# pouyaardehkhani/4DLangSplat

Measured on AMD Instinct MI355X. Metric: rasterizer fwd+bwd frames/sec @ 2M Gaussians, 1352x1014, 32-ch features, higher is better.
Workload: dtype f32; 1 GPU; S2M synthetic (BASELINE configs[2] per GPU; configs[3] batch split); gaussians=2000000, width=1352, height=1014, channels=32, global_batch=8, parallelism=dp1, pipeline=batched, binning=sort, early_views=2, order_on_side=True, num_rendered_mean=5615889

## Files before the change

4dlangsplat_amd/csrc/lsr_api.hip:

```cpp
#include <hip/hip_runtime.h>

#include <atomic>
#include <cstdio>
#include <cstring>
#include <mutex>
#include <string>
#include <vector>

#include "../../include/lsr.h"
#include "lsr_common.h"
#include "lsr_internal.h"

namespace {

thread_local std::string g_err;
std::atomic<int32_t> g_caller_api{0};

int fail(int code, const std::string& msg) {
    g_err = msg;
    return code;
}

#define LSR_HIP(expr)                                                                        \
    do {                                                                                     \
// ... 132 lines not shown
    BinningTb t;
    t.b = carve_binning(base, K, &head);
    Carver c(base);
    c.off = head;
    t.table = c.take<uint32_t>((size_t)lsr::tb_blocks((int)P) * ntiles);
    t.tmp = c.take<uint64_t>(K);
    if (bytes) *bytes = c.off;
    return t;
}

struct Img {
    uint2* ranges;
    uint32_t* tile_max;
    float* final_T;
    uint32_t* n_contrib;
    uint32_t* tile_order;
};
struct Grid { int x, y; size_t tiles() const { return (size_t)x * y; } };
Grid tile_grid(int W, int H) { return {(W + LSR_TILE_X - 1) / LSR_TILE_X, (H + LSR_TILE_Y - 1) / LSR_TILE_Y}; }
float focal(int extent, float tanfov) { return (float)extent / (2.0f * tanfov); }

Img carve_img(void* base, int W, int H, size_t* bytes) {
    const size_t ntiles = tile_grid(W, H).tiles();
    Carver c(base);
    Img m;
    m.ranges = c.take<uint2>(ntiles);
    m.tile_max = c.take<uint32_t>(ntiles);
    m.final_T = c.take<float>((size_t)W * H);
    m.n_contrib = c.take<uint32_t>((size_t)W * H);
    m.tile_order = c.take<uint32_t>(ntiles);
    if (bytes) *bytes = c.off;
    return m;
}

struct Scratch {
    float* acc_small;
    float* rec;
    uint8_t* flags;
};
Scratch carve_scratch(void* base, size_t P, size_t K, int recq, bool det, size_t* bytes) {
    Carver c(base);
    Scratch s{};
    if (det) {
        s.rec = c.take<float>(K * (size_t)recq);
        s.flags = c.take<uint8_t>(K);
    } else {
        s.acc_small = c.take<float>(P * lsr::ACC_PITCH);
    }
    if (bytes) *bytes = c.off;
    return s;
}

int tile_bits(int ntiles) {
    int b = 1;
    while ((1 << b) <= ntiles) ++b;
    return b;
}
bool tile_sort_in_b(int ntiles) { return ((tile_bits(ntiles) + 7) / 8) % 2 == 1; }
uint32_t* point_list(const Binning& b, Grid grid) { return tile_sort_in_b((int)grid.tiles()) ? b.val_b : b.val_a; }
int depth_sort_result_in_b() { return 0; }

int check_common(const lsr_settings* s, const lsr_fwd_in* in) {
    if (g_caller_api.load() != LSR_API_VERSION)
        return fail(LSR_EINVAL, "call lsr_require_api(LSR_API_VERSION) first: the caller must be built against lsr.h "
                                "version " + std::to_string(LSR_API_VERSION));
    if (!s || !in) return fail(LSR_EINVAL, "null settings or inputs");
    if (s->image_width <= 0 || s->image_height <= 0) return fail(LSR_EINVAL, "image size must be positive");
    if (s->image_width > 4095 * LSR_TILE_X || s->image_height > 4095 * LSR_TILE_Y)
        return fail(LSR_EINVAL, "image size exceeds 4095 tiles per axis");
    if (in->P < 0) return fail(LSR_EINVAL, "P must be >= 0");
    if (in->P >= (1 << 28)) return fail(LSR_EINVAL, "P must be < 2^28");
    if ((uint64_t)in->P * (uint64_t)(in->C > 16 ? in->C : 16) * 4u >= (1ull << 32))
        return fail(LSR_EINVAL, "P * max(C, 16) * 4 bytes must be < 2^32");
    if (!s->viewmatrix || !s->projmatrix || !s->bg || !s->campos)
        return fail(LSR_EINVAL, "viewmatrix, projmatrix, bg and campos are required");
    if (in->P > 0 && (!in->means3D || !in->opacities)) return fail(LSR_EINVAL, "means3D and opacities are required");
    if (in->P == 0) return LSR_OK;
    if ((in->shs == nullptr) == (in->colors_precomp == nullptr))
        return fail(LSR_EINVAL, "Please provide excatly one of either SHs or precomputed colors!");
    const bool sr = in->scales != nullptr || in->rotations != nullptr;
    if ((!(in->scales && in->rotations) && !in->cov3D_precomp) || (sr && in->cov3D_precomp))
        return fail(LSR_EINVAL, "Please provide exactly one of either scale/rotation pair or precomputed 3D covariance!");
    if (in->shs && (s->sh_degree < 0 || s->sh_degree > 3 || in->M < (s->sh_degree + 1) * (s->sh_degree + 1)))
        return fail(LSR_EINVAL, "sh_degree must be in [0, 3] and shs must hold (sh_degree + 1)^2 coefficients");
    if (in->C < 0 || in->C > 64) return fail(LSR_EINVAL, "language feature channels must be in [0, 64]");
    if (s->include_feature && in->C > 0 && in->P > 0 && !in->language_feature)
        return fail(LSR_EINVAL, "language_feature is required when C > 0");
    return LSR_OK;
}

enum : unsigned { SHARE_SIZE = 1, SHARE_SH_DEGREE = 2, SHARE_SCALE = 4, SHARE_FEATURE = 8 };
struct ViewRules { const char *no_views, *null_array; unsigned share; const char* share_msg; bool share_first; };
const char kArrays[] = "n_views >= 1 and the per-view arrays are required";
const ViewRules kPreprocessViews{kArrays, kArrays, SHARE_SIZE | SHARE_SH_DEGREE | SHARE_SCALE,
                                 "batched views must share the image size, sh_degree and scale_modifier", false};
const ViewRules kBinningViews{kArrays, kArrays, SHARE_SIZE, "batched views must share the image size", true};
const ViewRules kCompositeViews{kArrays, kArrays, SHARE_SIZE | SHARE_FEATURE,
                                "batched views must share the image size and include_feature", false};
const ViewRules kBackwardViews{"n_views must be >= 1", "null argument", SHARE_SCALE,
                               "all views must share scale_modifier", false};

bool shares(const lsr_settings* a, const lsr_settings* b, unsigned what) {
    return (!(what & SHARE_SIZE) || (a->image_width == b->image_width && a->image_height == b->image_height)) &&
           (!(what & SHARE_SH_DEGREE) || a->sh_degree == b->sh_degree) &&
           (!(what & SHARE_SCALE) || a->scale_modifier == b->scale_modifier) &&
           (!(what & SHARE_FEATURE) || (a->include_feature != 0) == (b->include_feature != 0));
}

template <typename Need>
int check_each_view(const ViewRules& rules, int32_t n_views, bool arrays, const lsr_settings* const* s,
                    const lsr_fwd_in* in, Need need) {
    if (n_views < 1) return fail(LSR_EINVAL, rules.no_views);
    if (!arrays) return fail(LSR_EINVAL, rules.null_array);
    for (int v = 0; v < n_views; ++v) {
        int rc = check_common(s[v], in);
        if (rc) return rc;
        if (rules.share_first && !shares(s[v], s[0], rules.share)) return fail(LSR_EINVAL, rules.share_msg);
        if ((rc = need(v))) return rc;
        if (!rules.share_first && !shares(s[v], s[0], rules.share)) return fail(LSR_EINVAL, rules.share_msg);
    }
    return LSR_OK;
}
int need_radii(int32_t n_views, lsr_fwd_out* const* out, int P) {
    for (int v = 0; v < n_views; ++v)
        if (!out[v] || (!out[v]->radii && P > 0)) return fail(LSR_EINVAL, "radii output is required");
    return LSR_OK;
}
int need_workspaces(const void* geom, const void* img, const void* binning, int64_t num_rendered) {
    if (!geom || !img || (num_rendered > 0 && !binning)) return fail(LSR_EINVAL, "workspaces are required");
    return LSR_OK;
}
int need_atomic_grads(const lsr_bwd_in* gin, const char* color_msg, const char* deterministic_msg) {
    if (!gin || !gin->dL_dout_color) return fail(LSR_EINVAL, color_msg);
    if (gin->deterministic) return fail(LSR_EINVAL, deterministic_msg);
    return LSR_OK;
}

void preprocess_shared(lsr::PreprocessArgs& a, const lsr_settings* s, const lsr_fwd_in* in) {
    const int W = s->image_width, H = s->image_height;
    const Grid grid = tile_grid(W, H);
    a.P = in->P; a.M = in->M; a.deg = s->sh_degree; a.W = W; a.H = H;
    a.grid_x = grid.x; a.grid_y = grid.y;
    a.scale_modifier = s->scale_modifier;
    a.means3D = in->means3D; a.scales = in->scales; a.rotations = in->rotations; a.opacities = in->opacities;
    a.shs = in->shs; a.colors_precomp = in->colors_precomp; a.cov3D_precomp = in->cov3D_precomp;
}
void preprocess_view(lsr::PreprocessView& v, const lsr_settings* s, const Geom& g, int* radii) {
    v.tanfovx = s->tanfovx; v.tanfovy = s->tanfovy;
    v.focal_x = focal(s->image_width, s->tanfovx);
    v.focal_y = focal(s->image_height, s->tanfovy);
    v.view = s->viewmatrix; v.proj = s->projmatrix; v.campos = s->campos;
    v.radii = radii; v.radius = g.radius; v.tiles = g.tiles; v.rect = g.rect; v.key = g.key_a; v.xy = g.xy;
    v.conic_o = g.conic_o; v.rgbd = g.rgbd; v.clamped = g.clamped;
    v.order = g.val_a;
    v.rank_counts = g.counts;
    v.acc = g.acc;
    v.clear.p[0] = g.total;
    v.clear.n[0] = 4;
}

uint32_t* mapped_counts(uint32_t* host_counts) {
    void* dptr = nullptr;
    if (hipHostGetDevicePointer(&dptr, host_counts, 0) == hipSuccess && dptr) return static_cast<uint32_t*>(dptr);
    (void)hipGetLastError();
    return nullptr;
}

int scan_counts(int nv, void* const* geom, int P, uint32_t* host_counts, uint32_t* mapped, hipStream_t st, bool debug) {
    lsr::ScanSeg sc[lsr::LSR_MAX_VIEWS] = {};
    const uint32_t* total[lsr::LSR_MAX_VIEWS];
    for (int k = 0; k < nv; ++k) {
        Geom g = carve_geom(geom[k], (size_t)P, nullptr);
        sc[k] = lsr::ScanSeg{g.counts, g.offsets, g.total, reinterpret_cast<uint32_t*>(g.scan_tmp), (size_t)P};
        total[k] = g.total;
        if (mapped) {
            sc[k].host_total = mapped + 2 * k;
            host_counts[2 * k + 1] = 0;
        }
    }
    uint32_t wrote;
    {
        PhaseTimer t(LSR_PHASE_INSTANCE_SCAN, st);
        wrote = lsr::exclusive_scan_batch(sc, nv, st);
    }
    LSR_LAUNCHED("instance scan", st, debug);
    for (int k = 0; k < nv; ++k)
        if (!((wrote >> k) & 1u))
            LSR_HIP(hipMemcpyAsync(host_counts + 2 * k, total[k], 2 * sizeof(uint32_t), hipMemcpyDeviceToHost, st));
    return LSR_OK;
}

struct BinBatch { int P, W, H; Grid grid; size_t ntiles; hipStream_t st; bool debug; };
struct BinView { Geom g; Img m; size_t K; void* binning; };
template <typename Launch>
int bin_views(int32_t n_views, const lsr_settings* const* s, const lsr_fwd_in* in, void* const* geom,
              void* const* binning, void* const* img, const int64_t* num_rendered, lsr_stream_t stream,
              size_t max_tiles, const char* too_many_tiles, Launch launch) {
    int rc = check_each_view(kBinningViews, n_views, s && geom && binning && img && num_rendered, s, in, [&](int v) {
        return need_workspaces(geom[v], img[v], binning[v], num_rendered[v]);
    });
    if (rc) return rc;
    const Grid grid = tile_grid(s[0]->image_width, s[0]->image_height);
    const BinBatch c{in->P, s[0]->image_width, s[0]->image_height, grid, grid.tiles(),
                     reinterpret_cast<hipStream_t>(stream), s[0]->debug != 0};
    if (c.ntiles > max_tiles) return fail(LSR_EINVAL, too_many_tiles);
    for (int v0 = 0; v0 < n_views; v0 += lsr::LSR_MAX_VIEWS) {
        const int nv = std::min(n_views - v0, lsr::LSR_MAX_VIEWS);
        BinView bv[lsr::LSR_MAX_VIEWS];
        int ne = 0;
        for (int v = v0; v < v0 + nv; ++v) {
            const size_t K = (size_t)num_rendered[v];
            Geom g = carve_geom(geom[v], (size_t)(c.P > 0 ? c.P : 1), nullptr);
            Img m = carve_img(img[v], c.W, c.H, nullptr);
            if (K == 0) {
                LSR_HIP(hipMemsetAsync(m.ranges, 0, sizeof(uint2) * c.ntiles, c.st));
                LSR_HIP(hipMemsetAsync(m.tile_max, 0, sizeof(uint32_t) * c.ntiles, c.st));
                continue;
            }
            bv[ne++] = BinView{g, m, K, binning[v]};
        }
        if (ne == 0) continue;
        if ((rc = launch(c, bv, ne))) return rc;
    }
    return LSR_OK;
}

void render_bwd_view(lsr::RenderBwdArgs& r, const lsr_settings* s, const lsr_fwd_in* in, const lsr_bwd_in* gin,
                     const Geom& g, const Binning& b, const Img& m) {
    const int W = s->image_width, H = s->image_height;
    const Grid grid = tile_grid(W, H);
    r.W = W; r.H = H; r.grid_x = grid.x; r.grid_y = grid.y; r.C = in->C; r.include_feature = s->include_feature;
    r.ranges = m.ranges; r.point_list = point_list(b, grid);
    r.xy = g.xy; r.conic_o = g.conic_o; r.rgbd = g.rgbd;
    r.rect = g.rect; r.inst_off = g.inst_off;
    r.lang = in->language_feature;
    r.lang_split = in->C == 32 ? in->language_feature_split : nullptr;
    r.bg = s->bg; r.final_T = m.final_T; r.n_contrib = m.n_contrib;
    r.tile_max_contrib = m.tile_max; r.tile_order = m.tile_order;
    r.dL_dcolor = gin->dL_dout_color; r.dL_dlang = gin->dL_dout_language_feature; r.dL_ddepth = gin->dL_dout_depth;
}

}

extern "C" {
namespace {
int check_views(int32_t n_views, const lsr_settings* const* s, const lsr_fwd_in* in, void* const* geom) {
    return check_each_view(kPreprocessViews, n_views, s && geom, s, in,
                           [&](int v) { return geom[v] ? LSR_OK : fail(LSR_EINVAL, "geom workspaces are required"); });
}

int preprocess_rows(int32_t n_views, int32_t row0, int32_t row1, int counts_tiles, const lsr_settings* const* s,
                    const lsr_fwd_in* in, lsr_fwd_out* const* out, void* const* geom, hipStream_t st) {
    const int P = in->P;
    if (row1 == row0) return LSR_OK;
    for (int v0 = 0; v0 < n_views; v0 += lsr::LSR_MAX_VIEWS) {
        const int nv = std::min(n_views - v0, lsr::LSR_MAX_VIEWS);
        lsr::PreprocessArgs a{};
        preprocess_shared(a, s[v0], in);
        a.nv = nv;
        a.row0 = row0;
        a.P = row1;
        a.counts_tiles = counts_tiles;
        for (int k = 0; k < nv; ++k) {
            Geom g = carve_geom(geom[v0 + k], (size_t)P, nullptr);
            preprocess_view(a.v[k], s[v0 + k], g, out[v0 + k]->radii);
        }
        {
            PhaseTimer t(LSR_PHASE_PREPROCESS, st);
            lsr::launch_preprocess(a, st);
        }
        LSR_LAUNCHED("preprocess", st, s[v0]->debug);
    }
    return LSR_OK;
}

int depth_order_views(int32_t n_views, const lsr_settings* const* s, const lsr_fwd_in* in, void* const* geom,
                      uint32_t* host_counts, uint32_t* mapped, hipStream_t st) {
    const int P = in->P;
    for (int v0 = 0; v0 < n_views; v0 += lsr::LSR_MAX_VIEWS) {
        const int nv = std::min(n_views - v0, lsr::LSR_MAX_VIEWS);
        lsr::SortSeg ss[lsr::LSR_MAX_VIEWS] = {};
        for (int k = 0; k < nv; ++k) {
            Geom g = carve_geom(geom[v0 + k], (size_t)P, nullptr);
            ss[k] = lsr::SortSeg{g.key_a, g.val_a, g.key_b, g.val_b, g.sort_tmp, g.total + 3,
                                 lsr::SortGather{g.rect, g.counts, g.rect_sorted}, (size_t)P};
            ss[k].vals_c = g.offsets;
        }
        {
            PhaseTimer t(LSR_PHASE_DEPTH_SORT, st);
            if (lsr::radix_sort_batch(ss, nv, 0, 32, st) != depth_sort_result_in_b())
                return fail(LSR_EHIP, "internal: depth sort batch or parity");
        }
        LSR_LAUNCHED("depth sort", st, s[v0]->debug);
        int rc = scan_counts(nv, geom + v0, P, host_counts + 2 * v0, mapped ? mapped + 2 * v0 : nullptr, st,
                             s[v0]->debug);
        if (rc) return rc;
    }
    return LSR_OK;
}

int instance_scan_views(int32_t n_views, const lsr_fwd_in* in, void* const* geom, uint32_t* host_counts,
                        uint32_t* mapped, hipStream_t st, bool debug) {
    for (int v0 = 0; v0 < n_views; v0 += lsr::LSR_MAX_VIEWS) {
        int rc = scan_counts(std::min(n_views - v0, lsr::LSR_MAX_VIEWS), geom + v0, in->P, host_counts + 2 * v0,
                             mapped ? mapped + 2 * v0 : nullptr, st, debug);
        if (rc) return rc;
    }
    return LSR_OK;
}
}
}

namespace {
int preprocess_and_order(int32_t n_views, int32_t n_ordered, const lsr_settings* const* s, const lsr_fwd_in* in,
                         lsr_fwd_out* const* out, void* const* geom, uint32_t* host_counts, bool map_counts,
                         hipStream_t st) {
    if (in->P == 0) {
        for (int v = 0; v < 2 * n_ordered; ++v) host_counts[v] = 0;
        return LSR_OK;
    }
    int rc = preprocess_rows(n_views, 0, in->P, 0, s, in, out, geom, st);
    if (rc || n_ordered == 0) return rc;
    return depth_order_views(n_ordered, s, in, geom, host_counts, map_counts ? mapped_counts(host_counts) : nullptr, st);
}

int preprocess_rows_checked(int32_t n_views, int32_t row0, int32_t row1, int counts_tiles, const lsr_settings* const* s,
                            const lsr_fwd_in* in, lsr_fwd_out* const* out, void* const* geom, lsr_stream_t stream) {
    int rc = check_views(n_views, s, in, geom);
    if (rc) return rc;
    if (!out || row0 < 0 || row1 < row0 || row1 > in->P || row0 % 256 != 0)
        return fail(LSR_EINVAL, "0 <= row0 <= row1 <= P with row0 a multiple of 256, and the outputs are required");
    if ((rc = need_radii(n_views, out, in->P))) return rc;
    return preprocess_rows(n_views, row0, row1, counts_tiles, s, in, out, geom, reinterpret_cast<hipStream_t>(stream));
}

int count_views(int32_t n_views, const lsr_settings* const* s, const lsr_fwd_in* in, void* const* geom,
                uint32_t* host_counts, lsr_stream_t stream, bool depth_sort) {
    int rc = check_views(n_views, s, in, geom);
    if (rc) return rc;
    if (!host_counts) return fail(LSR_EINVAL, "host_counts is required");
    if (in->P == 0) {
        for (int v = 0; v < 2 * n_views; ++v) host_counts[v] = 0;
        return LSR_OK;
    }
    hipStream_t st = reinterpret_cast<hipStream_t>(stream);
    uint32_t* mapped = mapped_counts(host_counts);
    return depth_sort ? depth_order_views(n_views, s, in, geom, host_counts, mapped, st)
                      : instance_scan_views(n_views, in, geom, host_counts, mapped, st, s[0]->debug);
}

lsr::PreprocessBwdViewsArgs preprocess_bwd_args(const lsr_settings* s, const lsr_fwd_in* in, const lsr_bwd_out* gout,
                                                size_t r0, int n, int nv) {
    lsr::PreprocessBwdViewsArgs a{};
    a.P = n; a.M = in->M; a.nv = nv; a.scale_modifier = s->scale_modifier;
    a.means3D = in->means3D + 3 * r0;
    a.scales = in->scales ? in->scales + 3 * r0 : nullptr;
    a.rotations = in->rotations ? in->rotations + 4 * r0 : nullptr;
    a.shs = in->shs ? in->shs + (size_t)in->M * 3 * r0 : nullptr;
    a.cov3D_precomp = in->cov3D_precomp ? in->cov3D_precomp + 6 * r0 : nullptr;
    a.dopacity = gout->dL_dopacity;
    a.dmeans3D = gout->dL_dmeans3D; a.dmeans2D = gout->dL_dmeans2D; a.dcolors = gout->dL_dcolors;
    a.dcov3D = gout->dL_dcov3D; a.dsh = in->shs ? gout->dL_dsh : nullptr; a.dscales = gout->dL_dscales;
    a.drots = gout->dL_drotations;
    return a;
}
void view_cam(lsr::ViewCam& c, const lsr_settings* s, const Geom& g, const float* acc_small, size_t r0) {
    c.view = s->viewmatrix; c.proj = s->projmatrix; c.campos = s->campos;
    c.tanfovx = s->tanfovx; c.tanfovy = s->tanfovy;
    c.focal_x = focal(s->image_width, s->tanfovx);
    c.focal_y = focal(s->image_height, s->tanfovy);
    c.deg = s->sh_degree;
    c.tiles = g.tiles + r0; c.clamped = g.clamped + r0;
    c.acc_small = acc_small + lsr::ACC_PITCH * r0;
}

}

extern "C" {

int lsr_version(void) { return LSR_API_VERSION; }
int lsr_require_api(int32_t caller_version) {
    if (caller_version != LSR_API_VERSION)
        return fail(LSR_EINVAL, "lsr.h version mismatch: caller " + std::to_string(caller_version) + ", library " +
                                    std::to_string(LSR_API_VERSION));
    g_caller_api.store(caller_version);
    return LSR_OK;
}
const char* lsr_last_error(void) { return g_err.c_str(); }

int64_t lsr_geom_bytes(int32_t P) {
    size_t b;
    carve_geom(nullptr, (size_t)(P > 0 ? P : 1), &b);
    return (int64_t)b;
}
int64_t lsr_binning_bytes(int64_t K) {
    size_t b;
    carve_binning(nullptr, (size_t)(K > 0 ? K : 1), &b);
    return (int64_t)b;
}
int64_t lsr_binning_bytes_tb(int64_t K, int32_t P, int32_t W, int32_t H) {
    if (W <= 0 || H <= 0 || P < 0) return -1;
    size_t b;
    carve_binning_tb(nullptr, (size_t)(K > 0 ? K : 1), (size_t)(P > 0 ? P : 1), tile_grid(W, H).tiles(), &b);
    return (int64_t)b;
}
int64_t lsr_img_bytes(int32_t W, int32_t H) {
    size_t b;
    carve_img(nullptr, W, H, &b);
    return (int64_t)b;
}
int64_t lsr_backward_bytes(int32_t P, int64_t K, int32_t C, int32_t deterministic) {
    size_t b;
    carve_scratch(nullptr, (size_t)(P > 0 ? P : 1), (size_t)(K > 0 ? K : 1), lsr::record_floats(C > 0 ? C : 0),
                  deterministic != 0, &b);
    return (int64_t)b;
}

int lsr_forward_preprocess_async(const lsr_settings* s, const lsr_fwd_in* in, lsr_fwd_out* out, void* geom,
                                 uint32_t* host_count, lsr_stream_t stream) {
    int rc = check_common(s, in);
    if (rc) return rc;
    if ((rc = need_radii(1, &out, in->P))) return rc;
    if (!geom || !host_count) return fail(LSR_EINVAL, "geom workspace and host_count are required");
    return preprocess_and_order(1, 1, &s, in, &out, &geom, host_count, false, reinterpret_cast<hipStream_t>(stream));
}

int lsr_forward_preprocess_views_split_async(int32_t n_views, int32_t n_ordered, const lsr_settings* const* s,
                                             const lsr_fwd_in* in, lsr_fwd_out* const* out, void* const* geom,
                                             uint32_t* host_counts, lsr_stream_t stream) {
    int rc = check_views(n_views, s, in, geom);
    if (rc) return rc;
    if (!out || (n_ordered > 0 && !host_counts) || n_ordered < 0 || n_ordered > n_views)
        return fail(LSR_EINVAL, "0 <= n_ordered <= n_views, the outputs and host_counts are required");
    if ((rc = need_radii(n_views, out, in->P))) return rc;
    return preprocess_and_order(n_views, n_ordered, s, in, out, geom, host_counts, true,
                                reinterpret_cast<hipStream_t>(stream));
}

int lsr_forward_preprocess_views_rows_async(int32_t n_views, int32_t row0, int32_t row1, const lsr_settings* const* s,
                                            const lsr_fwd_in* in, lsr_fwd_out* const* out, void* const* geom,
                                            lsr_stream_t stream) {
    return preprocess_rows_checked(n_views, row0, row1, 0, s, in, out, geom, stream);
}

int lsr_forward_preprocess_views_tb_async(int32_t n_views, int32_t row0, int32_t row1, const lsr_settings* const* s,
                                          const lsr_fwd_in* in, lsr_fwd_out* const* out, void* const* geom,
                                          lsr_stream_t stream) {
    return preprocess_rows_checked(n_views, row0, row1, 1, s, in, out, geom, stream);
}

int lsr_forward_instance_scan_views_async(int32_t n_views, const lsr_settings* const* s, const lsr_fwd_in* in,
                                          void* const* geom, uint32_t* host_counts, lsr_stream_t stream) {
    return count_views(n_views, s, in, geom, host_counts, stream, false);
}

int lsr_forward_depth_order_views_async(int32_t n_views, const lsr_settings* const* s, const lsr_fwd_in* in,
                                        void* const* geom, uint32_t* host_counts, lsr_stream_t stream) {
    return count_views(n_views, s, in, geom, host_counts, stream, true);
}

int lsr_forward_preprocess_views_async(int32_t n_views, const lsr_settings* const* s, const lsr_fwd_in* in,
                                       lsr_fwd_out* const* out, void* const* geom, uint32_t* host_counts,
                                       lsr_stream_t stream) {
    if (!host_counts) return fail(LSR_EINVAL, "host_counts is required");
    return lsr_forward_preprocess_views_split_async(n_views, n_views, s, in, out, geom, host_counts, stream);
}

int lsr_forward_preprocess(const lsr_settings* s, const lsr_fwd_in* in, lsr_fwd_out* out, void* geom,
                           int64_t* num_rendered, lsr_stream_t stream) {
    if (!num_rendered) return fail(LSR_EINVAL, "geom workspace and num_rendered are required");
    uint32_t tot[2] = {0, 0};
    int rc = lsr_forward_preprocess_async(s, in, out, geom, tot, stream);
    if (rc) return rc;
    LSR_HIP(hipStreamSynchronize(reinterpret_cast<hipStream_t>(stream)));
    *num_rendered = (int64_t)tot[0];
    return LSR_OK;
}

int lsr_forward_binning(const lsr_settings* s, const lsr_fwd_in* in, void* geom, void* binning, void* img,
                        int64_t num_rendered, lsr_stream_t stream) {
    return lsr_forward_binning_views(1, &s, in, &geom, &binning, &img, &num_rendered, stream);
}

int lsr_forward_binning_views(int32_t n_views, const lsr_settings* const* s, const lsr_fwd_in* in, void* const* geom,
                              void* const* binning, void* const* img, const int64_t* num_rendered,
                              lsr_stream_t stream) {
    const auto emit_and_sort = [](const BinBatch& c, const BinView* bv, int ne) {
        const size_t ntiles = c.ntiles;
        hipStream_t st = c.st;
        lsr::EmitBatch eb{};
        eb.P = c.P; eb.grid_x = c.grid.x; eb.grid_y = c.grid.y; eb.W = c.W; eb.H = c.H;
        lsr::SortSeg ss[lsr::LSR_MAX_VIEWS] = {};
        for (int k = 0; k < ne; ++k) {
            const Geom& g = bv[k].g;
            const Img& m = bv[k].m;
            Binning b = carve_binning(bv[k].binning, bv[k].K, nullptr);
            lsr::EmitView& e = eb.v[k];
            e.order = g.val_a; e.offsets = g.offsets; e.counts = g.counts; e.rect_sorted = g.rect_sorted;
            e.xy = g.xy; e.conic_o = g.conic_o; e.keys = b.key_a; e.vals = b.val_a;
            e.clear.p[0] = reinterpret_cast<uint32_t*>(m.ranges);
            e.clear.n[0] = (uint32_t)(2 * ntiles);
            e.clear.even[0] = 0xFFFFFFFFu;
            e.clear.p[1] = m.tile_max;
            e.clear.n[1] = (uint32_t)ntiles;
            ss[k] = lsr::SortSeg{b.key_a, b.val_a, b.key_b, b.val_b, b.sort_tmp, b.kept,
                                 lsr::SortGather{nullptr, nullptr, nullptr}, bv[k].K, m.ranges, (uint32_t)ntiles};
        }
        {
            PhaseTimer t(LSR_PHASE_EMIT, st);
            lsr::launch_emit_instances(eb, ne, st);
        }
        LSR_LAUNCHED("emit", st, c.debug);
        {
            PhaseTimer t(LSR_PHASE_TILE_SORT, st);
            const int in_b = lsr::radix_sort_batch(ss, ne, 0, tile_bits((int)ntiles), st);
            if (in_b < 0 || (in_b == 1) != tile_sort_in_b((int)ntiles))
                return fail(LSR_EHIP, "internal: tile sort batch or parity");
        }
        LSR_LAUNCHED("tile sort", st, c.debug);
        return LSR_OK;
    };
    return bin_views(n_views, s, in, geom, binning, img, num_rendered, stream, SIZE_MAX, nullptr, emit_and_sort);
}

int lsr_forward_binning_views_tb(int32_t n_views, const lsr_settings* const* s, const lsr_fwd_in* in, void* const* geom,
                                 void* const* binning, void* const* img, const int64_t* num_rendered,
                                 lsr_stream_t stream) {
    const auto bucket = [](const BinBatch& c, const BinView* bv, int ne) {
        lsr::TbBatch tb{};
        tb.P = c.P; tb.grid_x = c.grid.x; tb.grid_y = c.grid.y; tb.W = c.W; tb.H = c.H; tb.ntiles = (int)c.ntiles;
        for (int k = 0; k < ne; ++k) {
            const Geom& g = bv[k].g;
            const Img& m = bv[k].m;
            BinningTb b = carve_binning_tb(bv[k].binning, bv[k].K, (size_t)c.P, c.ntiles, nullptr);
            lsr::TbView& t = tb.v[k];
            t.counts = g.counts; t.offsets = g.offsets; t.rect = g.rect; t.xy = g.xy; t.conic_o = g.conic_o;
            t.depth = g.key_a;
            t.table = b.table;
            t.tile_total = m.tile_order;
            t.tile_start = m.tile_max;
            t.ranges = m.ranges;
            t.keys = reinterpret_cast<uint64_t*>(b.b.key_a);
            t.tmp = b.tmp;
            t.words = point_list(b.b, c.grid);
            t.tile_max = m.tile_max;
        }
        {
            PhaseTimer t(LSR_PHASE_TILE_SORT, c.st);
            const hipError_t e = lsr::launch_tile_bucket_binning(tb, ne, c.st);
            if (e != hipSuccess)
                return fail(LSR_EHIP, std::string("tile-bucket binning: dynamic LDS attribute: ") + hipGetErrorString(e));
        }
        LSR_LAUNCHED("tile-bucket binning", c.st, c.debug);
        return LSR_OK;
    };
    return bin_views(n_views, s, in, geom, binning, img, num_rendered, stream, 12288,
                     "tile-bucket binning: more than 12288 tiles (use lsr_forward_binning_views)", bucket);
}

int lsr_forward_composite(const lsr_settings* s, const lsr_fwd_in* in, lsr_fwd_out* out, const void* geom,
                          const void* binning, void* img, int64_t num_rendered, lsr_stream_t stream) {
    lsr_fwd_out* o[1] = {out};
    return lsr_forward_composite_views(1, &s, in, o, &geom, &binning, &img, &num_rendered, stream);
}

int lsr_forward_composite_views(int32_t n_views, const lsr_settings* const* s, const lsr_fwd_in* in,
                                lsr_fwd_out* const* out, const void* const* geom, const void* const* binning,
                                void* const* img, const int64_t* num_rendered, lsr_stream_t stream) {
    int rc = check_each_view(kCompositeViews, n_views, s && out && geom && binning && img && num_rendered, s, in, [&](int v) {
        if (!out[v] || !out[v]->out_color || !out[v]->out_depth) return fail(LSR_EINVAL, "color and depth outputs are required");
        if (in->C > 0 && !out[v]->out_language_feature)
            return fail(LSR_EINVAL, "language feature output is required when C > 0");
        return need_workspaces(geom[v], img[v], binning[v], num_rendered[v]);
    });
    if (rc) return rc;
    hipStream_t st = reinterpret_cast<hipStream_t>(stream);
    const int P = in->P, W = s[0]->image_width, H = s[0]->image_height, C = in->C;
    const Grid grid = tile_grid(W, H);
    for (int v0 = 0; v0 < n_views; v0 += lsr::LSR_MAX_VIEWS) {
        const int nv = std::min(n_views - v0, lsr::LSR_MAX_VIEWS);
        lsr::RenderFwdArgs r[lsr::LSR_MAX_VIEWS] = {};
        for (int k = 0; k < nv; ++k) {
            const int v = v0 + k;
            const size_t K = (size_t)num_rendered[v];
            Geom g = carve_geom(const_cast<void*>(geom[v]), (size_t)(P > 0 ? P : 1), nullptr);
            Binning b = carve_binning(const_cast<void*>(binning[v]), K > 0 ? K : 1, nullptr);
            Img m = carve_img(img[v], W, H, nullptr);
            lsr::RenderFwdArgs& a = r[k];
            a.W = W; a.H = H; a.grid_x = grid.x; a.grid_y = grid.y; a.C = C; a.include_feature = s[v]->include_feature;
            a.ranges = m.ranges; a.point_list = K > 0 ? point_list(b, grid) : nullptr;
            a.xy = g.xy; a.conic_o = g.conic_o; a.rgbd = g.rgbd;
            a.lang = in->language_feature;
            a.lang_split = in->C == 32 ? in->language_feature_split : nullptr;
            a.bg = s[v]->bg; a.final_T = m.final_T; a.n_contrib = m.n_contrib;
            a.tile_max_contrib = m.tile_max; a.tile_order = m.tile_order;
            a.out_color = out[v]->out_color; a.out_lang = out[v]->out_language_feature;
            a.out_depth = out[v]->out_depth;
            if (C > 0 && !s[v]->include_feature)
                LSR_HIP(hipMemsetAsync(out[v]->out_language_feature, 0, sizeof(float) * (size_t)C * W * H, st));
        }
        {
// ... 256 lines not shown
```

4dlangsplat_amd/csrc/lsr_internal.h:

```cpp
#pragma once
#include <hip/hip_runtime.h>
#include <stdint.h>

namespace lsr {

constexpr int ACC_PITCH = 16;

struct ClearList {
    uint32_t* p[4];
    uint32_t n[4];
    uint32_t even[4];
};

constexpr int LSR_MAX_VIEWS = 8;
__device__ __forceinline__ void clear_words(const ClearList& c) {
    const uint32_t t = blockIdx.x * blockDim.x + threadIdx.x, stride = gridDim.x * blockDim.x;
#pragma unroll
    for (int k = 0; k < 4; ++k)
        for (uint32_t i = t; i < c.n[k]; i += stride) c.p[k][i] = (i & 1u) ? 0u : c.even[k];
}

__host__ __device__ __forceinline__ uint2 rect_pack(uint32_t x0, uint32_t y0, uint32_t x1, uint32_t y1, uint32_t map) {
    return make_uint2(x0 | y0 << 12 | (map & 0xFFu) << 24, x1 | y1 << 12 | (map >> 8) << 24);
}
__host__ __device__ __forceinline__ void rect_unpack(uint2 r, uint32_t& x0, uint32_t& y0, uint32_t& x1, uint32_t& y1) {
    x0 = r.x & 0xFFFu; y0 = (r.x >> 12) & 0xFFFu; x1 = r.y & 0xFFFu; y1 = (r.y >> 12) & 0xFFFu;
}
__host__ __device__ __forceinline__ uint32_t rect_quad_map(uint2 r) { return (r.x >> 24) | (r.y >> 24) << 8; }
__host__ __device__ __forceinline__ bool rect_small(uint32_t x0, uint32_t y0, uint32_t x1, uint32_t y1) {
    return x1 - x0 <= 2 && y1 - y0 <= 2;
}
__host__ __device__ __forceinline__ uint32_t rect_tile_mask(uint32_t map) {
    return ((map & 0x33u) ? 1u : 0u) | ((map & 0xCCu) ? 2u : 0u) | ((map & 0x3300u) ? 4u : 0u) |
           ((map & 0xCC00u) ? 8u : 0u);
}
__host__ __device__ __forceinline__ uint32_t rect_count(uint2 r) {
    uint32_t x0, y0, x1, y1;
    rect_unpack(r, x0, y0, x1, y1);
    if ((x1 - x0) * (y1 - y0) > 0 && rect_small(x0, y0, x1, y1)) return __builtin_popcount(rect_tile_mask(rect_quad_map(r)));
    return (x1 - x0) * (y1 - y0);
}
__host__ __device__ __forceinline__ uint32_t rect_local_index(uint2 r, uint32_t tx, uint32_t ty) {
    uint32_t x0, y0, x1, y1;
    rect_unpack(r, x0, y0, x1, y1);
    if (rect_small(x0, y0, x1, y1))
        return __builtin_popcount(rect_tile_mask(rect_quad_map(r)) & ((1u << (2 * (ty - y0) + (tx - x0))) - 1u));
    return (ty - y0) * (x1 - x0) + (tx - x0);
}

struct PreprocessView {
    float tanfovx, tanfovy, focal_x, focal_y;
    const float* view;
    const float* proj;
    const float* campos;
    int* radii;
    int* radius;
    uint32_t* tiles;
    uint2* rect;
    uint32_t* key;
    float2* xy;
    float4* conic_o;
    float4* rgbd;
    uint8_t* clamped;
    uint32_t* order;
    uint32_t* rank_counts;
    float4* acc;
    ClearList clear;
};
struct PreprocessArgs {
    int P, M, deg, W, H, grid_x, grid_y, nv;
    int row0;
    int counts_tiles;
    float scale_modifier;
    const float* means3D;
    const float* scales;
    const float* rotations;
    const float* opacities;
    const float* shs;
    const float* colors_precomp;
    const float* cov3D_precomp;
    PreprocessView v[LSR_MAX_VIEWS];
};

struct ViewCam {
    const float* view;
    const float* proj;
    const float* campos;
    float tanfovx, tanfovy, focal_x, focal_y;
    int deg;
    const uint32_t* tiles;
    const uint8_t* clamped;
    const float* acc_small;
};
struct PreprocessBwdViewsArgs {
    int P, M, nv;
    float scale_modifier;
    const float* means3D;
    const float* scales;
    const float* rotations;
    const float* shs;
    const float* cov3D_precomp;
    ViewCam cam[LSR_MAX_VIEWS];
    float* dopacity;
    float* dmeans3D;
    float* dmeans2D;
    float* dcolors;
    float* dcov3D;
    float* dsh;
    float* dscales;
    float* drots;
    const float* rec;
    const uint8_t* flags;
    const uint32_t* inst_off;
    int recq;
    int deterministic;
};
void launch_preprocess_bwd_views(const PreprocessBwdViewsArgs& a, bool accumulate, bool one_view, hipStream_t st);

void launch_language_split(int P, const float* lang, uint16_t* out, hipStream_t st);
void launch_radii_max(int P, int n, const int* const* radii, int* out, bool accumulate, hipStream_t st);

struct RenderFwdArgs {
    int W, H, grid_x, grid_y, C, include_feature;
    uint2* ranges;
    const uint32_t* point_list;
    const float2* xy;
    const float4* conic_o;
    const float4* rgbd;
    const float* lang;
    const uint16_t* lang_split;
    const float* bg;
    float* final_T;
    uint32_t* n_contrib;
    uint32_t* tile_max_contrib;
    uint32_t* tile_order;
    float* out_color;
    float* out_lang;
    float* out_depth;
};

struct RenderBwdArgs {
    int W, H, grid_x, grid_y, C, include_feature;
    const uint2* ranges;
    const uint32_t* point_list;
    const float2* xy;
    const float4* conic_o;
    const float4* rgbd;
    const uint2* rect;
    const uint32_t* inst_off;
    const float* lang;
    const uint16_t* lang_split;
    const float* bg;
    const float* final_T;
    const uint32_t* n_contrib;
    const uint32_t* tile_max_contrib;
    uint32_t* tile_order;
    const float* dL_dcolor;
    const float* dL_dlang;
    const float* dL_ddepth;
    float* rec;
    uint8_t* flags;
    int recq;
    int deterministic;
    float* acc_small;
    float* acc_lang;
};

struct RenderFwdBatch { RenderFwdArgs v[LSR_MAX_VIEWS]; };
struct RenderBwdBatch { RenderBwdArgs v[LSR_MAX_VIEWS]; };
void launch_render_fwd_views(const RenderFwdArgs* a, int n, hipStream_t st);
void launch_render_bwd_wave_views(const RenderBwdArgs* a, int n, hipStream_t st);

inline int lang_pad(int C) { return C == 0 ? 0 : C <= 4 ? 4 : C <= 8 ? 8 : C <= 16 ? 16 : C <= 32 ? 32 : 64; }
inline int record_floats(int C) { return 12 + lang_pad(C); }

constexpr int DEF_MAX_LAYERS = 4;
constexpr int DEF_HEADS = 6;
constexpr int DEF_W2ROWS = 64;
constexpr int DEF_LANG_MODE_PASS = 0, DEF_LANG_MODE_RESIDUAL = 1, DEF_LANG_MODE_NORESNET = 2,
              DEF_LANG_MODE_DISCRETE = 3;
struct DeformArgs {
    int P;
    int n_scales, nlayers;
    uint32_t heads;
    int apply_rotation, lang_mode, lang_dim, centers, lang_in;
    const float* means3D;
    const float* time;
    const float* aabb;
    const float* planes;
    int64_t poff[24];
    int pw[24], ph[24];
    const __bf16 *wf_h[DEF_MAX_LAYERS], *wf_l[DEF_MAX_LAYERS];
    const __bf16 *w1_h[DEF_HEADS], *w1_l[DEF_HEADS];
    const __bf16 *w2_h[DEF_HEADS], *w2_l[DEF_HEADS];
    const float* b_feat[DEF_MAX_LAYERS];
    const float* b1[DEF_HEADS];
    const float* b2[DEF_HEADS];
    const float* in[5];
    const float* lang;
    float* out[5];
    float* out_lang;
    float* out_coff;
};
void launch_deform_fwd(const DeformArgs& a, hipStream_t st);
enum PackKind { PACK_PLANE = 0, PACK_WEIGHT = 1, PACK_WEIGHT_T = 2 };
struct PackJob {
    int kind, a, b, c, d;
    uint32_t first_block;
    const float* src;
    void* hi;
    __bf16* lo;
};
constexpr int PACK_MAX_JOBS = 64;
struct PackBatch { PackJob j[PACK_MAX_JOBS]; int n; };
void launch_pack_batch(PackJob* jobs, int n, hipStream_t st);

struct DeformBwdArgs {
    DeformArgs f;
    const __bf16 *wft_h[DEF_MAX_LAYERS], *wft_l[DEF_MAX_LAYERS];
    const __bf16 *w1t_h[DEF_HEADS], *w1t_l[DEF_HEADS];
    const __bf16 *w2t_h[DEF_HEADS], *w2t_l[DEF_HEADS];
    const float* up[5];
    const float* up_lang;
    const float* up_coff;
    float* d_means3D;
    float* d_rotations;
    float* d_lang;
    float* dplanes;
    int64_t plane_stride;
    int replicas;
    float* trow;
    int64_t toff[24];
    int64_t trow_stride;
    int trow_reps;
    float* sX;
    float* sA[DEF_MAX_LAYERS];
    float* sdH[DEF_MAX_LAYERS];
    float* sG_rot;
    float* sG_coff;
    float* daabb;
    float* daabb_part;
};
constexpr int DEF_AABB_SLOTS = 64;
void launch_deform_bwd_a(const DeformBwdArgs& a, hipStream_t st);
struct HeadWgradJob {
    const float* G;
    const __bf16 *w1_h, *w1_l;
    const float* b1;
    const __bf16 *w2t_h, *w2t_l;
    const __bf16 *w2_h, *w2_l;
    float *dW1, *db1, *dW2, *db2;
    int nout;
};
constexpr int DEF_WGRAD_MAX_JOBS = DEF_HEADS;
struct HeadWgradArgs {
    HeadWgradJob job[DEF_WGRAD_MAX_JOBS];
    const float* A;
    int P, rows_per_block;
};
void launch_head_wgrad(const HeadWgradArgs& a, int njobs, hipStream_t st);
struct AtbJob {
    const float* L;
    const float* R;
    float* C;
    float* bias;
    int M, N;
};
constexpr int LSR_ATB_MAX_JOBS = 20;
struct AtbArgs {
    AtbJob job[LSR_ATB_MAX_JOBS];
    int P;
    int rows_per_block;
};
void launch_atb(const AtbArgs& a, int njobs, hipStream_t st);
constexpr int DEF_UNPACK_MAX = 24;
struct UnpackBatch {
    const float* src;
    int64_t off[DEF_UNPACK_MAX];
    float* dst[DEF_UNPACK_MAX];
    int H[DEF_UNPACK_MAX], W[DEF_UNPACK_MAX];
    int block0[DEF_UNPACK_MAX + 1];
    int n, replicas;
    int64_t stride;
    const float* daabb_part;
    float* daabb;
    const float* trow;
    int64_t toff[DEF_UNPACK_MAX];
    int64_t trow_stride;
    int trow_reps;
    const float* time0;
};
void launch_unpack_planes(const UnpackBatch& u, hipStream_t st);

struct LangDeformArgs {
    int P, lang_dim, time_pe, kin, residual;
    const float* lang;
    const float* time;
    const __bf16 *w_h[3], *w_l[3];
    const float* b[3];
    float* out_lang;
    const __bf16 *wt_h[3], *wt_l[3];
    const float* up_lang;
    float* d_lang;
    float *sU0, *sU1, *sU2;
    float *sdv, *sdZ2, *sdZ1;
};
void launch_lang_deform_fwd(const LangDeformArgs& a, hipStream_t st);
void launch_lang_deform_bwd(const LangDeformArgs& a, hipStream_t st);

void launch_preprocess(const PreprocessArgs& a, hipStream_t st);
void launch_reduce_lang(int P, int C, int cpad, int recq, const float* rec, const uint8_t* flags,
                        const uint32_t* inst_off, const uint32_t* tiles, float* dlang, bool accumulate, hipStream_t st);
void launch_mark_visible(int P, const float* means3D, const float* view, uint8_t* present, hipStream_t st);

size_t scan_temp_bytes(size_t n);
void exclusive_scan_u32(const uint32_t* in, uint32_t* out, size_t n, uint32_t* total, void* temp, hipStream_t st);
constexpr int SCAN_SEG_TILES = 4096;
struct ScanSeg {
    const uint32_t* in;
    uint32_t* out;
    uint32_t* total;
    uint32_t* partials;
    size_t n;
    uint32_t* host_total = nullptr;
};
struct ScanBatch { ScanSeg s[LSR_MAX_VIEWS]; };
uint32_t exclusive_scan_batch(const ScanSeg* segs, int nseg, hipStream_t st);
size_t radix_temp_bytes(size_t n);
struct SortGather {
    const uint2* rect;
    uint32_t* counts;
    uint2* rect_sorted;
};
struct SortSeg {
    uint32_t *keys_a, *vals_a, *keys_b, *vals_b;
    void* temp;
    uint32_t* kept;
    SortGather gather;
    size_t n;
    uint2* ranges;
    uint32_t nranges;
    uint32_t* vals_c;
};
struct SortBatch { SortSeg s[LSR_MAX_VIEWS]; };
int radix_sort_batch(const SortSeg* segs, int nseg, int begin_bit, int end_bit, hipStream_t st);
bool radix_sort_pairs(uint32_t* keys_a, uint32_t* vals_a, uint32_t* keys_b, uint32_t* vals_b, size_t n,
                      int begin_bit, int end_bit, void* temp, hipStream_t st, uint32_t* kept = nullptr,
                      const SortGather* gather = nullptr, uint32_t* vals_c = nullptr);

constexpr uint32_t PL_ID_MASK = 0x0FFFFFFFu;
constexpr int PL_QUAD_SHIFT = 28;
struct EmitView {
    const uint32_t* order;
    const uint32_t* offsets;
    const uint32_t* counts;
    const uint2* rect_sorted;
    const float2* xy;
    const float4* conic_o;
    uint32_t* keys;
    uint32_t* vals;
    ClearList clear;
};
struct EmitBatch {
    int P, grid_x, grid_y, W, H;
    EmitView v[LSR_MAX_VIEWS];
};
void launch_emit_instances(const EmitBatch& eb, int nv, hipStream_t st);
void launch_scatter_inst_off(int P, const uint32_t* order, const uint32_t* offsets, const uint32_t* counts,
                             uint32_t* inst_off, hipStream_t st);
struct TbView {
    const uint32_t* counts;
    const uint32_t* offsets;
    const uint2* rect;
    const float2* xy;
    const float4* conic_o;
    const uint32_t* depth;
    uint32_t* table;
    uint32_t* tile_total;
    uint32_t* tile_start;
    uint2* ranges;
    uint64_t* keys;
    uint64_t* tmp;
    uint32_t* words;
    uint32_t* tile_max;
};
struct TbBatch {
    int P, grid_x, grid_y, W, H, ntiles;
    TbView v[LSR_MAX_VIEWS];
};
int tb_blocks(int P);
hipError_t launch_tile_bucket_binning(const TbBatch& tb, int nv, hipStream_t st);

void launch_render_bwd(const RenderBwdArgs& a, hipStream_t st);
void launch_render_fwd_wave_views(const RenderFwdArgs* a, int n, hipStream_t st);
void launch_render_fwd_wave_mfma_views(const RenderFwdArgs* a, int n, hipStream_t st);

}
```

4dlangsplat_amd/csrc/preprocess.hip:

```cpp
#include "lsr_common.h"
#include "lsr_internal.h"

namespace lsr {

struct m3 { float m[3][3]; };

__device__ __forceinline__ m3 mul(const m3& a, const m3& b) {
    m3 o;
#pragma unroll
    for (int c = 0; c < 3; ++c)
#pragma unroll
        for (int r = 0; r < 3; ++r)
            o.m[c][r] = a.m[0][r] * b.m[c][0] + a.m[1][r] * b.m[c][1] + a.m[2][r] * b.m[c][2];
    return o;
}
__device__ __forceinline__ m3 tr(const m3& a) {
    m3 o;
#pragma unroll
    for (int c = 0; c < 3; ++c)
#pragma unroll
        for (int r = 0; r < 3; ++r) o.m[c][r] = a.m[r][c];
    return o;
}
__device__ __forceinline__ m3 quat_R(float4 q) {
    const float r = q.x, x = q.y, y = q.z, z = q.w;
    m3 R;
    R.m[0][0] = 1.0f - 2.0f * (y * y + z * z); R.m[0][1] = 2.0f * (x * y - r * z); R.m[0][2] = 2.0f * (x * z + r * y);
    R.m[1][0] = 2.0f * (x * y + r * z); R.m[1][1] = 1.0f - 2.0f * (x * x + z * z); R.m[1][2] = 2.0f * (y * z - r * x);
    R.m[2][0] = 2.0f * (x * z - r * y); R.m[2][1] = 2.0f * (y * z + r * x); R.m[2][2] = 1.0f - 2.0f * (x * x + y * y);
    return R;
}
__device__ __forceinline__ m3 zero3() {
    m3 o;
#pragma unroll
    for (int c = 0; c < 3; ++c)
#pragma unroll
        for (int r = 0; r < 3; ++r) o.m[c][r] = 0.0f;
    return o;
}

__device__ __forceinline__ void cov3d(float3 s, float mod, float4 q, float* cov) {
    m3 S = zero3();
    S.m[0][0] = mod * s.x; S.m[1][1] = mod * s.y; S.m[2][2] = mod * s.z;
    const m3 Rm = quat_R(q);
    const m3 M = mul(S, Rm);
    const m3 Sig = mul(tr(M), M);
    cov[0] = Sig.m[0][0]; cov[1] = Sig.m[0][1]; cov[2] = Sig.m[0][2];
    cov[3] = Sig.m[1][1]; cov[4] = Sig.m[1][2]; cov[5] = Sig.m[2][2];
}

__device__ __forceinline__ m3 view_W(const float* __restrict__ v) {
    m3 W;
    W.m[0][0] = v[0]; W.m[0][1] = v[4]; W.m[0][2] = v[8];
    W.m[1][0] = v[1]; W.m[1][1] = v[5]; W.m[1][2] = v[9];
    W.m[2][0] = v[2]; W.m[2][1] = v[6]; W.m[2][2] = v[10];
    return W;
}
__device__ __forceinline__ m3 sym3(const float* c) {
    m3 V;
    V.m[0][0] = c[0]; V.m[0][1] = c[1]; V.m[0][2] = c[2];
    V.m[1][0] = c[1]; V.m[1][1] = c[3]; V.m[1][2] = c[4];
    V.m[2][0] = c[2]; V.m[2][1] = c[4]; V.m[2][2] = c[5];
    return V;
}

__constant__ float SH_C0 = 0.28209479177387814f;
__constant__ float SH_C1 = 0.4886025119029199f;
__constant__ float SH_C2[5] = {1.0925484305920792f, -1.0925484305920792f, 0.31539156525252005f,
                               -1.0925484305920792f, 0.5462742152960396f};
__constant__ float SH_C3[7] = {-0.5900435899266435f, 2.890611442640554f, -0.4570457994644658f,
                               0.3731763325901154f, -0.4570457994644658f, 1.445305721320277f,
                               -0.5900435899266435f};

template <int M3>
__device__ __forceinline__ void stage_rows(float* __restrict__ lds, const float* __restrict__ src, int rows) {
    if constexpr (M3 > 0) {
        constexpr int SP = M3 + 1;
        const int n = rows * M3;
        for (int e = threadIdx.x; e < n; e += blockDim.x) {
            const int r = e / M3, c = e - r * M3;
            lds[r * SP + c] = src[e];
        }
    }
}

template <int MS>
struct GaussIn {
    float3 p;
    float op;
    float c3[6];
    float sh[MS > 0 ? 3 * MS : 1];
};
__device__ __forceinline__ float3 load_mean(const PreprocessArgs& a, int i) {
    return make_float3(a.means3D[3 * i], a.means3D[3 * i + 1], a.means3D[3 * i + 2]);
}
__device__ __forceinline__ void load_cov3d(const PreprocessArgs& a, int i, float (&c3)[6]) {
    if (a.cov3D_precomp) {
#pragma unroll
        for (int k = 0; k < 6; ++k) c3[k] = a.cov3D_precomp[6 * (size_t)i + k];
    } else {
        const float3 s = make_float3(a.scales[3 * i], a.scales[3 * i + 1], a.scales[3 * i + 2]);
        const float4 q = reinterpret_cast<const float4*>(a.rotations)[i];
        cov3d(s, a.scale_modifier, q, c3);
    }
}
template <int MS, int N>
__device__ __forceinline__ void load_sh(const PreprocessArgs& a, int i, float (&shr)[N]) {
    constexpr int M3 = MS * 3;
    const float* src = a.shs + (size_t)i * M3;
    if (M3 % 4 == 0 && (reinterpret_cast<uintptr_t>(src) & 15) == 0) {
#pragma unroll
        for (int q = 0; q < M3 / 4; ++q) {
            const float4 t = reinterpret_cast<const float4*>(src)[q];
            shr[4 * q] = t.x; shr[4 * q + 1] = t.y; shr[4 * q + 2] = t.z; shr[4 * q + 3] = t.w;
        }
    } else {
#pragma unroll
        for (int q = 0; q < M3; ++q) shr[q] = src[q];
    }
}
template <int MS>
__device__ __forceinline__ void load_gauss(const PreprocessArgs& a, int i, GaussIn<MS>& g) {
    g.p = load_mean(a, i);
    g.op = a.opacities[i];
    load_cov3d(a, i, g.c3);
    if constexpr (MS > 0) {
        if (a.shs && !a.colors_precomp) load_sh<MS>(a, i, g.sh);
    }
}

template <int MS, bool PRE>
__device__ __forceinline__ bool preprocess_one(const PreprocessArgs& a, const PreprocessView& v, const GaussIn<MS>& g,
                                               int i) {
    v.radii[i] = 0;
    v.radius[i] = 0;
    v.tiles[i] = 0;
    v.rect[i] = make_uint2(0u, 0u);
    v.clamped[i] = 0;
    if (v.order) v.order[i] = (uint32_t)i;
    if (v.rank_counts) v.rank_counts[i] = 0u;
    if (v.key) v.key[i] = 0xFFFFFFFFu;
    const float3 p = PRE ? g.p : load_mean(a, i);
    const float4 ph = xform4x4(v.proj, p);
    const float3 pv = xform4x3(v.view, p);
    if (pv.z <= 0.2f) return false;
    const float pw = 1.0f / (ph.w + 0.0000001f);
    const float3 pp = make_float3(ph.x * pw, ph.y * pw, ph.z * pw);

    float c3[6];
    if constexpr (PRE) {
#pragma unroll
        for (int k = 0; k < 6; ++k) c3[k] = g.c3[k];
    } else {
        load_cov3d(a, i, c3);
    }
    float3 t = pv;
    const float limx = 1.3f * v.tanfovx, limy = 1.3f * v.tanfovy;
    const float txtz = t.x / t.z, tytz = t.y / t.z;
    t.x = fminf(limx, fmaxf(-limx, txtz)) * t.z;
    t.y = fminf(limy, fmaxf(-limy, tytz)) * t.z;
    m3 J = zero3();
    J.m[0][0] = v.focal_x / t.z; J.m[0][2] = -(v.focal_x * t.x) / (t.z * t.z);
    J.m[1][1] = v.focal_y / t.z; J.m[1][2] = -(v.focal_y * t.y) / (t.z * t.z);
    const m3 T = mul(view_W(v.view), J);
    const m3 V = sym3(c3);
    const m3 A = mul(tr(T), tr(V));
    const m3 cv = mul(A, T);
    const float ca = cv.m[0][0] + 0.3f, cb = cv.m[0][1], cc = cv.m[1][1] + 0.3f;
    const float det = ca * cc - cb * cb;
    if (det == 0.0f) return false;
    const float det_inv = 1.0f / det;
    const float4 conic = make_float4(cc * det_inv, -cb * det_inv, ca * det_inv, PRE ? g.op : a.opacities[i]);
    const float mid = 0.5f * (ca + cc);
    const float l1 = mid + sqrtf(fmaxf(0.1f, mid * mid - det));
    const float l2 = mid - sqrtf(fmaxf(0.1f, mid * mid - det));
    const int radius = (int)ceilf(3.0f * sqrtf(fmaxf(l1, l2)));
    const float2 pix = make_float2(ndc2pix(pp.x, a.W), ndc2pix(pp.y, a.H));
    int2 rmin, rmax;
    tile_rect(pix, radius, a.grid_x, a.grid_y, rmin, rmax);
    if ((rmax.y - rmin.y) * (rmax.x - rmin.x) == 0) return false;
    const float thr = skip_power(conic.w);
    int ntiles = 0;
    int2 cmin = make_int2(0, 0), cmax = make_int2(0, 0);
    if (thr <= 0.0f) {
        const float rr = (float)radius + 16.0f;
        const float mt = (fabsf(conic.x) + fabsf(conic.z) + 2.0f * fabsf(conic.y)) * rr * rr;
        const float qm = -2.0f * thr + 1e-6f * mt + 1e-4f;
        const float hx = sqrtf(qm * ca) + 0.01f, hy = sqrtf(qm * cc) + 0.01f;
        cmin.x = max(rmin.x, (int)floorf((pix.x - hx) / (float)LSR_TILE_X));
        cmin.y = max(rmin.y, (int)floorf((pix.y - hy) / (float)LSR_TILE_Y));
        cmax.x = min(rmax.x, (int)floorf((pix.x + hx) / (float)LSR_TILE_X) + 1);
        cmax.y = min(rmax.y, (int)floorf((pix.y + hy) / (float)LSR_TILE_Y) + 1);
        if (cmax.x > cmin.x && cmax.y > cmin.y) ntiles = (cmax.x - cmin.x) * (cmax.y - cmin.y);
        else cmin = cmax = make_int2(0, 0);
    }

    float rgb[3];
    if (a.colors_precomp) {
        rgb[0] = a.colors_precomp[3 * i]; rgb[1] = a.colors_precomp[3 * i + 1]; rgb[2] = a.colors_precomp[3 * i + 2];
    } else {
        float3 dir = make_float3(p.x - v.campos[0], p.y - v.campos[1], p.z - v.campos[2]);
        const float len = sqrtf(dir.x * dir.x + dir.y * dir.y + dir.z * dir.z);
        dir.x = dir.x / len; dir.y = dir.y / len; dir.z = dir.z / len;
        float shr[48];
        if constexpr (MS > 0) {
            if constexpr (PRE) {
#pragma unroll
                for (int q = 0; q < 3 * MS; ++q) shr[q] = g.sh[q];
            } else {
                load_sh<MS>(a, i, shr);
            }
        }
        const float* sh = MS > 0 ? shr : a.shs + (size_t)i * a.M * 3;
        uint8_t cl = 0;
        const int deg = a.deg;
#pragma unroll
        for (int ch = 0; ch < 3; ++ch) {
#define SHc(k) sh[(k) * 3 + ch]
            float res = SH_C0 * SHc(0);
            if (deg > 0) {
                const float x = dir.x, y = dir.y, z = dir.z;
                res = res - SH_C1 * y * SHc(1) + SH_C1 * z * SHc(2) - SH_C1 * x * SHc(3);
                if (deg > 1) {
                    const float xx = x * x, yy = y * y, zz = z * z, xy = x * y, yz = y * z, xz = x * z;
                    res = res + SH_C2[0] * xy * SHc(4) + SH_C2[1] * yz * SHc(5) +
                          SH_C2[2] * (2.0f * zz - xx - yy) * SHc(6) + SH_C2[3] * xz * SHc(7) +
                          SH_C2[4] * (xx - yy) * SHc(8);
                    if (deg > 2) {
                        res = res + SH_C3[0] * y * (3.0f * xx - yy) * SHc(9) + SH_C3[1] * xy * z * SHc(10) +
                              SH_C3[2] * y * (4.0f * zz - xx - yy) * SHc(11) +
                              SH_C3[3] * z * (2.0f * zz - 3.0f * xx - 3.0f * yy) * SHc(12) +
                              SH_C3[4] * x * (4.0f * zz - xx - yy) * SHc(13) + SH_C3[5] * z * (xx - yy) * SHc(14) +
                              SH_C3[6] * x * (xx - 3.0f * yy) * SHc(15);
                    }
                }
            }
#undef SHc
            res = res + 0.5f;
            cl |= (res < 0.0f ? 1 : 0) << ch;
            rgb[ch] = res < 0.0f ? 0.0f : res;
        }
        v.clamped[i] = cl;
    }
    v.radii[i] = radius;
    v.radius[i] = radius;
    uint32_t qmap = 0;
    if (ntiles > 0 && cmax.x - cmin.x <= 2 && cmax.y - cmin.y <= 2) {
        const EmitSplat es = emit_splat(pix, conic);
        const float ex = emit_margin(es);
        for (int ty = cmin.y; ty < cmax.y; ++ty)
#pragma unroll
            for (int band = 0; band < 2; ++band) {
                bool ok;
                float xmin, xmax;
                emit_band(es, ty * LSR_TILE_Y + 8 * band, a.H, ex, ok, xmin, xmax);
                for (int tx = cmin.x; tx < cmax.x; ++tx)
#pragma unroll
                    for (int col = 0; col < 2; ++col)
                        qmap |= emit_col_hit(es, ok, xmin, xmax, tx * LSR_TILE_X + 8 * col, a.W)
                                    ? 1u << (8 * (ty - cmin.y) + 4 * band + 2 * (tx - cmin.x) + col) : 0u;
            }
    }
    const uint2 rc = rect_pack((uint32_t)cmin.x, (uint32_t)cmin.y, (uint32_t)cmax.x, (uint32_t)cmax.y, qmap);
    v.rect[i] = rc;
    v.tiles[i] = rect_count(rc);
    if (v.rank_counts && a.counts_tiles) v.rank_counts[i] = rect_count(rc);
    if (v.key) v.key[i] = __float_as_uint(pv.z);
    v.xy[i] = pix;
    v.conic_o[i] = conic;
    v.rgbd[i] = make_float4(rgb[0], rgb[1], rgb[2], pv.z);
    return ntiles > 0;
}

__device__ __forceinline__ void zero_acc_rows(float4* acc, bool rect, int i) {
    if (!acc) return;
    const uint64_t m = __ballot(rect);
    if (m == 0) return;
    const int ln = threadIdx.x & 63;
    float4* w = acc + (size_t)(i - ln) * (ACC_PITCH / 4);
#pragma unroll
    for (int q = 0; q < ACC_PITCH / 4; ++q) {
        const int e = q * 64 + ln;
        if ((m >> (e / (ACC_PITCH / 4))) & 1) w[e] = make_float4(0.0f, 0.0f, 0.0f, 0.0f);
    }
}

template <int MS, bool MULTI>
__global__ void __launch_bounds__(256) k_preprocess(PreprocessArgs a) {
    const int i = a.row0 + blockIdx.x * blockDim.x + threadIdx.x;
    GaussIn<MS> g;
    if constexpr (!MULTI) {
        clear_words(a.v[0].clear);
        const bool rect = i < a.P && preprocess_one<MS, false>(a, a.v[0], g, i);
        zero_acc_rows(a.v[0].acc, rect, i);
    } else {
        const bool ok = i < a.P;
        if (ok) load_gauss<MS>(a, i, g);
        for (int k = 0; k < a.nv; ++k) {
            const PreprocessView& v = a.v[k];
            clear_words(v.clear);
            const bool rect = ok && preprocess_one<MS, true>(a, v, g, i);
            zero_acc_rows(v.acc, rect, i);
        }
    }
}

void launch_preprocess(const PreprocessArgs& a, hipStream_t st) {
    if (a.P <= a.row0 || a.nv <= 0) return;
    const dim3 grid((a.P - a.row0 + 255) / 256), block(256);
#define LSR_PP(MS)                                                                   \
    do {                                                                             \
        if (a.nv > 1) hipLaunchKernelGGL((k_preprocess<MS, true>), grid, block, 0, st, a);  \
        else hipLaunchKernelGGL((k_preprocess<MS, false>), grid, block, 0, st, a);          \
    } while (0)
    switch ((a.shs && !a.colors_precomp) ? a.M : 0) {
        case 1: LSR_PP(1); break;
        case 4: LSR_PP(4); break;
        case 9: LSR_PP(9); break;
        case 16: LSR_PP(16); break;
        default: LSR_PP(0); break;
    }
#undef LSR_PP
}

__global__ void k_mark_visible(int P, const float* __restrict__ means3D, const float* __restrict__ view,
                               uint8_t* __restrict__ present) {
    const int i = blockIdx.x * blockDim.x + threadIdx.x;
    if (i >= P) return;
    const float3 p = make_float3(means3D[3 * i], means3D[3 * i + 1], means3D[3 * i + 2]);
    present[i] = xform4x3(view, p).z > 0.2f;
}
struct RadiiMaxArgs { const int* r[LSR_MAX_VIEWS]; };
__global__ void __launch_bounds__(256) k_radii_max(int P, int n, RadiiMaxArgs ra, int* __restrict__ out, int accumulate) {
    const int i4 = blockIdx.x * 256 + threadIdx.x, i = 4 * i4;
    if (i >= P) return;
    if (i + 4 <= P) {
        int4 m = accumulate ? reinterpret_cast<const int4*>(out)[i4] : make_int4(0, 0, 0, 0);
        for (int v = 0; v < n; ++v) {
            const int4 x = reinterpret_cast<const int4*>(ra.r[v])[i4];
            m = make_int4(max(m.x, x.x), max(m.y, x.y), max(m.z, x.z), max(m.w, x.w));
        }
        reinterpret_cast<int4*>(out)[i4] = m;
    } else {
        for (int k = i; k < P; ++k) {
            int m = accumulate ? out[k] : 0;
            for (int v = 0; v < n; ++v) m = max(m, ra.r[v][k]);
            out[k] = m;
        }
    }
}
void launch_radii_max(int P, int n, const int* const* radii, int* out, bool accumulate, hipStream_t st) {
    for (int v0 = 0; v0 < n; v0 += LSR_MAX_VIEWS) {
        RadiiMaxArgs ra{};
        const int nv = n - v0 < LSR_MAX_VIEWS ? n - v0 : LSR_MAX_VIEWS;
        for (int k = 0; k < nv; ++k) ra.r[k] = radii[v0 + k];
        hipLaunchKernelGGL(k_radii_max, dim3((unsigned)((P + 1023) / 1024)), dim3(256), 0, st, P, nv, ra, out,
                           (accumulate || v0 > 0) ? 1 : 0);
    }
}

void launch_mark_visible(int P, const float* means3D, const float* view, uint8_t* present, hipStream_t st) {
    if (P == 0) return;
    hipLaunchKernelGGL(k_mark_visible, dim3((P + 255) / 256), dim3(256), 0, st, P, means3D, view, present);
}

__device__ void cov2d_bwd(float3 mean, const float* c3, float fx, float fy, float tanfovx, float tanfovy,
                          const float* __restrict__ view, float3 dconic, float3& dmean, float* dcov) {
#pragma clang fp contract(fast)
    float3 t = xform4x3(view, mean);
    const float limx = 1.3f * tanfovx, limy = 1.3f * tanfovy;
    const float txtz = t.x / t.z, tytz = t.y / t.z;
    t.x = fminf(limx, fmaxf(-limx, txtz)) * t.z;
    t.y = fminf(limy, fmaxf(-limy, tytz)) * t.z;
    const float x_grad_mul = (txtz < -limx || txtz > limx) ? 0.0f : 1.0f;
    const float y_grad_mul = (tytz < -limy || tytz > limy) ? 0.0f : 1.0f;
    const float tz = __builtin_amdgcn_rcpf(t.z), tz2 = tz * tz, tz3 = tz2 * tz;
    const float J00 = fx * tz, J11 = fy * tz, J02 = -(fx * t.x) * tz2, J12 = -(fy * t.y) * tz2;
    float u0[3], u1[3], Vu0[3], Vu1[3];
#pragma unroll
    for (int r = 0; r < 3; ++r) {
        u0[r] = view[4 * r] * J00 + view[4 * r + 2] * J02;
        u1[r] = view[4 * r + 1] * J11 + view[4 * r + 2] * J12;
    }
    const float V[3][3] = {{c3[0], c3[1], c3[2]}, {c3[1], c3[3], c3[4]}, {c3[2], c3[4], c3[5]}};
#pragma unroll
    for (int r = 0; r < 3; ++r) {
        Vu0[r] = V[r][0] * u0[0] + V[r][1] * u0[1] + V[r][2] * u0[2];
        Vu1[r] = V[r][0] * u1[0] + V[r][1] * u1[1] + V[r][2] * u1[2];
    }
    const float a = u0[0] * Vu0[0] + u0[1] * Vu0[1] + u0[2] * Vu0[2] + 0.3f;
    const float b = u0[0] * Vu1[0] + u0[1] * Vu1[1] + u0[2] * Vu1[2];
    const float c = u1[0] * Vu1[0] + u1[1] * Vu1[1] + u1[2] * Vu1[2] + 0.3f;
    const float denom = a * c - b * b;
    float dL_da = 0.0f, dL_db = 0.0f, dL_dc = 0.0f;
    const float denom2inv = __builtin_amdgcn_rcpf((denom * denom) + 0.0000001f);
    if (denom2inv != 0.0f) {
        dL_da = denom2inv * (-c * c * dconic.x + 2.0f * b * c * dconic.y + (denom - a * c) * dconic.z);
        dL_dc = denom2inv * (-a * a * dconic.z + 2.0f * a * b * dconic.y + (denom - a * c) * dconic.x);
        dL_db = denom2inv * 2.0f * (b * c * dconic.x - (denom + 2.0f * b * b) * dconic.y + a * b * dconic.z);
    }
    dcov[0] = u0[0] * u0[0] * dL_da + u0[0] * u1[0] * dL_db + u1[0] * u1[0] * dL_dc;
    dcov[3] = u0[1] * u0[1] * dL_da + u0[1] * u1[1] * dL_db + u1[1] * u1[1] * dL_dc;
    dcov[5] = u0[2] * u0[2] * dL_da + u0[2] * u1[2] * dL_db + u1[2] * u1[2] * dL_dc;
    dcov[1] = 2.0f * u0[0] * u0[1] * dL_da + (u0[0] * u1[1] + u0[1] * u1[0]) * dL_db + 2.0f * u1[0] * u1[1] * dL_dc;
    dcov[2] = 2.0f * u0[0] * u0[2] * dL_da + (u0[0] * u1[2] + u0[2] * u1[0]) * dL_db + 2.0f * u1[0] * u1[2] * dL_dc;
    dcov[4] = 2.0f * u0[2] * u0[1] * dL_da + (u0[1] * u1[2] + u0[2] * u1[1]) * dL_db + 2.0f * u1[1] * u1[2] * dL_dc;
    float dT0[3], dT1[3];
#pragma unroll
    for (int k = 0; k < 3; ++k) {
        dT0[k] = 2.0f * Vu0[k] * dL_da + Vu1[k] * dL_db;
        dT1[k] = 2.0f * Vu1[k] * dL_dc + Vu0[k] * dL_db;
    }
    const float dJ00 = view[0] * dT0[0] + view[4] * dT0[1] + view[8] * dT0[2];
    const float dJ02 = view[2] * dT0[0] + view[6] * dT0[1] + view[10] * dT0[2];
    const float dJ11 = view[1] * dT1[0] + view[5] * dT1[1] + view[9] * dT1[2];
    const float dJ12 = view[2] * dT1[0] + view[6] * dT1[1] + view[10] * dT1[2];
    const float dtx = x_grad_mul * -fx * tz2 * dJ02;
    const float dty = y_grad_mul * -fy * tz2 * dJ12;
    const float dtz = -fx * tz2 * dJ00 - fy * tz2 * dJ11 + (2.0f * fx * t.x) * tz3 * dJ02 + (2.0f * fy * t.y) * tz3 * dJ12;
    dmean.x = view[0] * dtx + view[1] * dty + view[2] * dtz;
    dmean.y = view[4] * dtx + view[5] * dty + view[6] * dtz;
    dmean.z = view[8] * dtx + view[9] * dty + view[10] * dtz;
}

__device__ void cov3d_bwd(float3 sc, float mod, float4 q, const float* dcov, float3& dscale, float4& drot) {
#pragma clang fp contract(fast)
    const float r = q.x, x = q.y, y = q.z, z = q.w;
    const m3 Rm = quat_R(q);
    const float s[3] = {mod * sc.x, mod * sc.y, mod * sc.z};
    m3 S = zero3();
    S.m[0][0] = s[0]; S.m[1][1] = s[1]; S.m[2][2] = s[2];
    const m3 M = mul(S, Rm);
    m3 dS;
    dS.m[0][0] = dcov[0]; dS.m[0][1] = 0.5f * dcov[1]; dS.m[0][2] = 0.5f * dcov[2];
    dS.m[1][0] = 0.5f * dcov[1]; dS.m[1][1] = dcov[3]; dS.m[1][2] = 0.5f * dcov[4];
    dS.m[2][0] = 0.5f * dcov[2]; dS.m[2][1] = 0.5f * dcov[4]; dS.m[2][2] = dcov[5];
    m3 M2;
#pragma unroll
    for (int c = 0; c < 3; ++c)
#pragma unroll
        for (int k = 0; k < 3; ++k) M2.m[c][k] = 2.0f * M.m[c][k];
    const m3 dM = mul(M2, dS);
    const m3 Rt = tr(Rm);
    m3 d = tr(dM);
    float ds[3];
#pragma unroll
    for (int k = 0; k < 3; ++k) ds[k] = (Rt.m[k][0] * d.m[k][0] + Rt.m[k][1] * d.m[k][1] + Rt.m[k][2] * d.m[k][2]) * mod;
    dscale = make_float3(ds[0], ds[1], ds[2]);
#pragma unroll
    for (int k = 0; k < 3; ++k) { d.m[0][k] *= s[0]; d.m[1][k] *= s[1]; d.m[2][k] *= s[2]; }
    drot.x = 2.0f * z * (d.m[0][1] - d.m[1][0]) + 2.0f * y * (d.m[2][0] - d.m[0][2]) + 2.0f * x * (d.m[1][2] - d.m[2][1]);
    drot.y = 2.0f * y * (d.m[1][0] + d.m[0][1]) + 2.0f * z * (d.m[2][0] + d.m[0][2]) + 2.0f * r * (d.m[1][2] - d.m[2][1]) -
             4.0f * x * (d.m[2][2] + d.m[1][1]);
    drot.z = 2.0f * x * (d.m[1][0] + d.m[0][1]) + 2.0f * r * (d.m[2][0] - d.m[0][2]) + 2.0f * z * (d.m[1][2] + d.m[2][1]) -
             4.0f * y * (d.m[2][2] + d.m[0][0]);
// ... 354 lines not shown
```

4dlangsplat_amd/csrc/sort.hip:

```cpp
#include "lsr_common.h"
#include "lsr_internal.h"

namespace lsr {

constexpr int SCAN_ITEMS = 8;
constexpr int SCAN_TILE = 256 * SCAN_ITEMS;

static inline size_t align_up(size_t x, size_t a) { return (x + a - 1) / a * a; }

__device__ __forceinline__ void block_exclusive_scan8(uint32_t (&v)[SCAN_ITEMS], uint32_t* s_wave,
                                                      uint32_t& block_total) {
    const int lane = threadIdx.x & 63, wave = threadIdx.x >> 6;
    uint32_t local = 0;
#pragma unroll
    for (int i = 0; i < SCAN_ITEMS; ++i) { const uint32_t x = v[i]; v[i] = local; local += x; }
    uint32_t inc = local;
#pragma unroll
    for (int o = 1; o < 64; o <<= 1) {
        const uint32_t t = __shfl_up(inc, o);
        if (lane >= o) inc += t;
    }
    if (lane == 63) s_wave[wave] = inc;
    __syncthreads();
    uint32_t wave_off = 0, total = 0;
// ... 271 lines not shown
    const uint64_t lt = lanemask_lt();
    const size_t base = (size_t)blockIdx.x * (256 * IT) + (size_t)wave * (64 * IT);
    uint32_t key[IT];
#pragma unroll
    for (int r = 0; r < IT; ++r) {
        const size_t idx = base + (size_t)r * 64 + lane;
        key[r] = idx < n ? keys[idx] : 0u;
    }
    uint32_t kmin = 0xFFFFFFFFu, kmax = 0u;
#pragma unroll
    for (int r = 0; r < IT; ++r) {
        const bool valid = base + (size_t)r * 64 + lane < n && !(drop && key[r] == 0xFFFFFFFFu);
        if (valid) {
            kmin = min(kmin, key[r]);
            kmax = max(kmax, key[r]);
        }
        const uint32_t d = ((key[r] - pd.kbase) >> pd.shift) & mask;
        const uint64_t peers = match_digit(d, valid, pd.nbits);
        if (valid && (peers & lt) == 0) s_h[wave][d] += (uint32_t)__popcll(peers);
        __builtin_amdgcn_wave_barrier();
    }
    const bool plan = sg.vals_c && pass == 0;
    if (plan) {
#pragma unroll
        for (int o = 32; o >= 1; o >>= 1) {
            kmin = min(kmin, (uint32_t)__shfl_xor((int)kmin, o));
            kmax = max(kmax, (uint32_t)__shfl_xor((int)kmax, o));
        }
        if (lane == 0) { s_mm[0][wave] = kmin; s_mm[1][wave] = kmax; }
    }
    __syncthreads();
    for (int d = tid; d < (1 << pd.nbits); d += 256)
        counts[(size_t)blockIdx.x * RDX + d] = s_h[0][d] + s_h[1][d] + s_h[2][d] + s_h[3][d];
    if (plan && tid < 2) {
        const uint32_t v = tid == 0 ? min(min(s_mm[0][0], s_mm[0][1]), min(s_mm[0][2], s_mm[0][3]))
                                    : max(max(s_mm[1][0], s_mm[1][1]), max(s_mm[1][2], s_mm[1][3]));
        counts[(size_t)blockIdx.x * RDX + 256 + tid] = v;
    }
}

constexpr int SCAN_ROWS = 8;
template <int DG>
__global__ void __launch_bounds__(256) k_rts_scan(const SortBatch b, int pass, int it, int in_b, int nbits_h) {
    constexpr int Q = DG / 4;
    __shared__ uint32_t s_part[4][DG];
    const SortSeg& sg = b.s[blockIdx.y];
    const PassDesc pd = pass_desc(sg, pass, in_b, 0, nbits_h, 0);
    if (!pd.active) return;
    const int nbits = pd.nbits;
    const int d0 = DG * (int)blockIdx.x, tid = threadIdx.x, lane = tid & 63, wave = tid >> 6;
    uint32_t* __restrict__ totals = rts_totals(sg, pass);
    const int nb = (int)rts_blocks(sg.n, it);
    uint32_t* __restrict__ counts = rts_rows(sg, pass, (size_t)nb);
    if (sg.vals_c && pass == 0 && blockIdx.x == 0) {
        uint32_t kmin = 0xFFFFFFFFu, kmax = 0u;
        for (int r = tid; r < nb; r += 256) {
            kmin = min(kmin, counts[(size_t)r * RDX + 256]);
            kmax = max(kmax, counts[(size_t)r * RDX + 257]);
        }
#pragma unroll
        for (int o = 32; o >= 1; o >>= 1) {
            kmin = min(kmin, (uint32_t)__shfl_xor((int)kmin, o));
            kmax = max(kmax, (uint32_t)__shfl_xor((int)kmax, o));
        }
        if (lane == 0) { s_part[0][wave] = kmin; s_part[1][wave] = kmax; }
        __syncthreads();
        if (tid == 0) {
            const uint32_t lo = min(min(s_part[0][0], s_part[0][1]), min(s_part[0][2], s_part[0][3]));
            const uint32_t hi = max(max(s_part[1][0], s_part[1][1]), max(s_part[1][2], s_part[1][3]));
            const uint32_t kbase = lo & ~0xFFu;
            const bool three = lo <= hi && hi - kbase < (1u << 26);
            uint32_t* pl = rts_plan(sg);
            pl[0] = three ? kbase : 0u;
            pl[1] = three ? 1u : 0u;
        }
        __syncthreads();
    }
    if (d0 >= (1 << nbits)) {
        if (tid < DG) totals[d0 + tid] = 0u;
        return;
    }
    uint32_t carry[DG];
#pragma unroll
    for (int j = 0; j < DG; ++j) carry[j] = 0u;
    for (int c0 = 0; c0 < nb; c0 += 256 * SCAN_ROWS) {
        const int r0 = c0 + tid * SCAN_ROWS;
        uint4 v[SCAN_ROWS][Q];
#pragma unroll
        for (int r = 0; r < SCAN_ROWS; ++r) {
            const uint4* p = reinterpret_cast<const uint4*>(counts + (size_t)(r0 + r) * RDX + d0);
#pragma unroll
            for (int q = 0; q < Q; ++q) v[r][q] = r0 + r < nb ? p[q] : make_uint4(0u, 0u, 0u, 0u);
        }
        uint32_t sum[DG];
#pragma unroll
        for (int q = 0; q < Q; ++q) {
            sum[4 * q] = 0u; sum[4 * q + 1] = 0u; sum[4 * q + 2] = 0u; sum[4 * q + 3] = 0u;
#pragma unroll
            for (int r = 0; r < SCAN_ROWS; ++r) {
                sum[4 * q] += v[r][q].x; sum[4 * q + 1] += v[r][q].y;
                sum[4 * q + 2] += v[r][q].z; sum[4 * q + 3] += v[r][q].w;
            }
        }
        uint32_t off[DG], tot[DG];
#pragma unroll
        for (int j = 0; j < DG; ++j) {
            uint32_t inc = sum[j];
#pragma unroll
            for (int o = 1; o < 64; o <<= 1) {
                const uint32_t t = __shfl_up(inc, o);
                if (lane >= o) inc += t;
            }
            off[j] = inc - sum[j];
            if (lane == 63) s_part[wave][j] = inc;
        }
        __syncthreads();
#pragma unroll
        for (int j = 0; j < DG; ++j) {
            uint32_t before = 0u, all = 0u;
#pragma unroll
            for (int w = 0; w < 4; ++w) {
                const uint32_t x = s_part[w][j];
                before += w < wave ? x : 0u;
                all += x;
            }
            off[j] += before + carry[j];
            tot[j] = all;
        }
#pragma unroll
        for (int r = 0; r < SCAN_ROWS; ++r) {
            if (r0 + r >= nb) break;
            uint4* p = reinterpret_cast<uint4*>(counts + (size_t)(r0 + r) * RDX + d0);
#pragma unroll
            for (int q = 0; q < Q; ++q) {
                const uint4 x = v[r][q];
                p[q] = make_uint4(off[4 * q], off[4 * q + 1], off[4 * q + 2], off[4 * q + 3]);
                off[4 * q] += x.x; off[4 * q + 1] += x.y; off[4 * q + 2] += x.z; off[4 * q + 3] += x.w;
            }
        }
#pragma unroll
        for (int j = 0; j < DG; ++j) carry[j] += tot[j];
        __syncthreads();
    }
    if (tid < DG) {
        uint32_t t = 0u;
#pragma unroll
        for (int j = 0; j < DG; ++j) t = tid == j ? carry[j] : t;
        totals[d0 + tid] = t;
    }
}

constexpr int SCAN_DG = 16;

template <int IT>
__global__ void __launch_bounds__(256) k_rts_scatter(const SortBatch b, int pass, int in_b, int shift, int nbits_h,
                                                     int last_h) {
    __shared__ uint32_t s_key[(256 * IT)];
    __shared__ uint32_t s_val[(256 * IT)];
    __shared__ uint32_t s_wcnt[4][RDX];
    __shared__ uint32_t s_gbase[RDX];
    __shared__ uint32_t s_lbase[RDX];
    __shared__ uint32_t s_wave[4];
    const SortSeg& sg = b.s[blockIdx.y];
    const size_t nbi = rts_blocks(sg.n, IT);
    const uint32_t bid = blockIdx.x;
    if (bid >= nbi) return;
    const PassDesc pd = pass_desc(sg, pass, in_b, shift, nbits_h, last_h);
    if (!pd.active) return;
    const uint32_t* __restrict__ keys_in = keys_of(sg, pd.src);
    const uint32_t* __restrict__ vals_in = vals_of(sg, pd.src);
    uint32_t* __restrict__ keys_out = keys_of_w(sg, pd.dst);
    uint32_t* __restrict__ vals_out = vals_of_w(sg, pd.dst);
    const int drop = sg.kept && pass == 0;
    uint32_t* kept_out = drop ? sg.kept : nullptr;
    const uint32_t* __restrict__ totals = rts_totals(sg, pass);
    const uint32_t* __restrict__ offs = rts_rows(sg, pass, nbi);
    const SortGather gather = pd.last ? sg.gather : SortGather{nullptr, nullptr, nullptr};
    const int tid = threadIdx.x, wave = tid >> 6, lane = tid & 63;
    const int nd = 1 << pd.nbits;
#pragma unroll
    for (int w = 0; w < 4; ++w) {
        s_wcnt[w][tid] = 0;
        s_wcnt[w][tid + 256] = 0;
    }
    const size_t n = rts_n(sg.n, sg.kept && pass > 0 ? sg.kept : nullptr);
    __syncthreads();
    const uint32_t mask = (uint32_t)nd - 1u;
    const uint64_t lt = lanemask_lt();
    const size_t base = (size_t)bid * (256 * IT) + (size_t)wave * (64 * IT);
    uint32_t key[IT], val[IT], rank[IT];
#pragma unroll
    for (int r = 0; r < IT; ++r) {
        const size_t idx = base + (size_t)r * 64 + lane;
        const bool valid = idx < n;
        key[r] = valid ? keys_in[idx] : 0u;
        val[r] = valid ? vals_in[idx] : 0u;
    }
    const int da = 2 * tid, db = 2 * tid + 1;
    const uint32_t pre_a = da < nd ? offs[(size_t)bid * RDX + da] : 0u, pre_b = db < nd ? offs[(size_t)bid * RDX + db] : 0u;
    const uint32_t hc_a = da < nd ? totals[da] : 0u, hc_b = db < nd ? totals[db] : 0u;
#pragma unroll
    for (int r = 0; r < IT; ++r) {
        const bool valid = base + (size_t)r * 64 + lane < n && !(drop && key[r] == 0xFFFFFFFFu);
        const uint32_t d = ((key[r] - pd.kbase) >> pd.shift) & mask;
        const uint64_t peers = match_digit(d, valid, pd.nbits);
        const uint32_t before = s_wcnt[wave][d];
        const uint32_t pr = (uint32_t)__popcll(peers & lt);
        rank[r] = before + pr;
        __builtin_amdgcn_wave_barrier();
        if (valid && pr == 0) s_wcnt[wave][d] = before + (uint32_t)__popcll(peers);
        __builtin_amdgcn_wave_barrier();
    }
    __syncthreads();
    uint32_t tot_a, tot_b;
    {
        const uint32_t a0 = s_wcnt[0][da], a1 = s_wcnt[1][da], a2 = s_wcnt[2][da], a3 = s_wcnt[3][da];
        const uint32_t b0 = s_wcnt[0][db], b1 = s_wcnt[1][db], b2 = s_wcnt[2][db], b3 = s_wcnt[3][db];
        tot_a = a0 + a1 + a2 + a3;
        tot_b = b0 + b1 + b2 + b3;
        s_wcnt[0][da] = 0; s_wcnt[1][da] = a0; s_wcnt[2][da] = a0 + a1; s_wcnt[3][da] = a0 + a1 + a2;
        s_wcnt[0][db] = 0; s_wcnt[1][db] = b0; s_wcnt[2][db] = b0 + b1; s_wcnt[3][db] = b0 + b1 + b2;
    }
    const uint32_t dstart_a = block_excl_scan256(hc_a + hc_b, s_wave);
    const uint32_t lbase_a = block_excl_scan256(tot_a + tot_b, s_wave);
    s_lbase[da] = lbase_a;
    s_lbase[db] = lbase_a + tot_a;
    s_gbase[da] = dstart_a + pre_a - lbase_a;
    s_gbase[db] = dstart_a + hc_a + pre_b - (lbase_a + tot_a);
    if (tid == 255) {
        s_wave[0] = lbase_a + tot_a + tot_b;
        if (kept_out && bid == 0) *kept_out = dstart_a + hc_a + hc_b;
    }
    __syncthreads();
    const int ntile = (int)s_wave[0];
#pragma unroll
    for (int r = 0; r < IT; ++r) {
        const bool valid = base + (size_t)r * 64 + lane < n && !(drop && key[r] == 0xFFFFFFFFu);
        if (valid) {
            const uint32_t d = ((key[r] - pd.kbase) >> pd.shift) & mask;
            const uint32_t pos = s_lbase[d] + s_wcnt[wave][d] + rank[r];
            s_key[pos] = key[r];
            s_val[pos] = val[r];
        }
    }
    __syncthreads();
    if (gather.rect) {
        uint2 rc[IT];
        uint32_t vv[IT], dd[IT];
#pragma unroll
        for (int r = 0; r < IT; ++r) {
            const int i = tid + 256 * r;
            const bool ok = i < ntile;
            const uint32_t k = s_key[ok ? i : 0], v = s_val[ok ? i : 0];
            vv[r] = v;
            dd[r] = s_gbase[((k - pd.kbase) >> pd.shift) & mask] + (uint32_t)i;
            rc[r] = ok ? gather.rect[v] : make_uint2(0u, 0u);
        }
#pragma unroll
        for (int r = 0; r < IT; ++r) {
            if (tid + 256 * r < ntile) {
                vals_out[dd[r]] = vv[r];
                gather.rect_sorted[dd[r]] = rc[r];
                gather.counts[dd[r]] = rect_count(rc[r]);
            }
        }
        return;
    }
    uint2* __restrict__ ranges = pd.last ? sg.ranges : nullptr;
    for (int i = tid; i < ntile; i += 256) {
        const uint32_t k = s_key[i];
        const uint32_t dst = s_gbase[((k - pd.kbase) >> pd.shift) & mask] + (uint32_t)i;
        keys_out[dst] = k;
        vals_out[dst] = s_val[i];
        if (ranges && k < sg.nranges) {
            if (i == 0 || s_key[i - 1] != k) atomicMin(&ranges[k].x, dst);
            if (i == ntile - 1 || s_key[i + 1] != k) atomicMax(&ranges[k].y, dst + 1u);
        }
    }
}

static size_t os_blocks(size_t n) { return (n + OS_TILE - 1) / OS_TILE; }

size_t radix_temp_bytes(size_t n) {
    return RTS_ROWS_OFF + align_up(4 * os_blocks(n) * RDX * 4, 256);
}

int radix_sort_batch(const SortSeg* segs, int nseg, int begin_bit, int end_bit, hipStream_t st) {
    SortBatch bt{};
    int ns = 0;
    size_t nmax = 0;
    for (int i = 0; i < nseg; ++i)
        if (segs[i].n > 0) { bt.s[ns++] = segs[i]; nmax = std::max(nmax, segs[i].n); }
    if (ns == 0 || end_bit <= begin_bit) return 0;
    for (int i = 1; i < ns; ++i)
        if ((bt.s[i].vals_c == nullptr) != (bt.s[0].vals_c == nullptr)) return -1;
    if (bt.s[0].vals_c && (begin_bit != 0 || end_bit != 32)) return -1;
    for (int i = 0; i < ns; ++i) {
        const SortSeg& g = bt.s[i];
        if (g.vals_c && !(g.kept && g.gather.rect && g.gather.counts && g.gather.rect_sorted)) return -1;
    }
    const int items = (nmax > ((size_t)4 << 20) || bt.s[0].vals_c) ? 12 : OS_ITEMS;
    const unsigned nbi = (unsigned)((nmax + 256 * items - 1) / (256 * items));
    auto pass = [&](int p, int in_b, int shift, int nbits, int last) {
        if (items == 12)
            hipLaunchKernelGGL(k_rts_count<12>, dim3(nbi, ns), dim3(256), 0, st, bt, p, in_b, shift, nbits);
        else
            hipLaunchKernelGGL(k_rts_count<OS_ITEMS>, dim3(nbi, ns), dim3(256), 0, st, bt, p, in_b, shift, nbits);
        hipLaunchKernelGGL(k_rts_scan<SCAN_DG>, dim3(RDX / SCAN_DG, ns), dim3(256), 0, st, bt, p, items, in_b, nbits);
        if (items == 12)
            hipLaunchKernelGGL(k_rts_scatter<12>, dim3(nbi, ns), dim3(256), 0, st, bt, p, in_b, shift, nbits, last);
        else
            hipLaunchKernelGGL(k_rts_scatter<OS_ITEMS>, dim3(nbi, ns), dim3(256), 0, st, bt, p, in_b, shift, nbits,
                               last);
    };
    if (bt.s[0].vals_c) {
        for (int p = 0; p < 4; ++p) pass(p, 0, 0, 8, 0);
        return 0;
    }
    bool in_b = false;
    const int npass = (end_bit - begin_bit + 7) / 8;
    for (int shift = begin_bit, nbits = 0, p = 0; shift < end_bit; shift += nbits, ++p) {
        nbits = (end_bit - begin_bit) / npass + (p < (end_bit - begin_bit) % npass ? 1 : 0);
        pass(p, (int)in_b, shift, nbits, shift + nbits >= end_bit);
        in_b = !in_b;
    }
    return in_b ? 1 : 0;
}

bool radix_sort_pairs(uint32_t* keys_a, uint32_t* vals_a, uint32_t* keys_b, uint32_t* vals_b, size_t n,
                      int begin_bit, int end_bit, void* temp, hipStream_t st, uint32_t* kept, const SortGather* gather,
                      uint32_t* vals_c) {
    if (n == 0 || end_bit <= begin_bit) return false;
    SortSeg sg{keys_a, vals_a, keys_b, vals_b, temp, kept, gather ? *gather : SortGather{nullptr, nullptr, nullptr}, n};
    sg.vals_c = (vals_c && kept && sg.gather.rect && sg.gather.counts && sg.gather.rect_sorted && begin_bit == 0 &&
                 end_bit == 32)
                    ? vals_c
                    : nullptr;
    return radix_sort_batch(&sg, 1, begin_bit, end_bit, st) == 1;
}

}
```

4dlangsplat_amd/diff_gaussian_rasterization/__init__.py:

```python
from __future__ import annotations

import ctypes
import functools
from typing import NamedTuple, Optional

import torch
import torch.nn as nn

from . import _lib

__all__ = ["GaussianRasterizationSettings", "GaussianRasterizer", "rasterize_gaussians", "RasterizerState",
           "forward_native", "backward_native", "backward_views_native", "backward_composite_native",
           "backward_preprocess_views_native", "preprocess_views_native", "binning_views_native",
           "render_views_native", "backward_composite_views_native", "language_split_native", "rasterize_views",
           "radii_max_native"]

_lib.load()
_BINNING_DELAY_CYCLES = 0


class GaussianRasterizationSettings(NamedTuple):
    image_height: int
    image_width: int
    tanfovx: float
# ... 72 lines not shown
    return ctypes.c_void_p(torch.cuda.current_stream(device).cuda_stream)


class PendingForward:

    def __init__(self, raster_settings, settings, fin, inputs, geom, radii, K, device, H, W):
        self.raster_settings, self.settings, self.fin, self.inputs = raster_settings, settings, fin, inputs
        self.geom, self.radii, self.num_rendered, self.device, self.H, self.W = geom, radii, K, device, H, W
        self.binning = self.img = None
        self.ready = None
        self.ready_stream = None
        self.count_host = None
        self.counted = None
        self.stream = None
        self.count_batch = None
        self.tile_bucket = False

    def resolve(self, binning=False):
        if self.counted is None:
            return self
        self.counted.synchronize()
        self.counted = None
        self.num_rendered = int(self.count_host[0])
        if binning:
            _run_binning(self, self.stream)
        return self


def _dump_forward(raster_settings, inputs):
    if raster_settings.debug:
        torch.save({k: (None if v is None else v.cpu()) for k, v in inputs.items()
                    if k in ("means3D", "opacities", "shs", "colors_precomp", "scales", "rotations")},
                   "snapshot_fw.dump")
        print("\nAn error occured in forward. Writing snapshot_fw.dump for debugging.")


def _check_forward(rc, what, raster_settings, inputs):
    try:
        _lib.check(rc, what)
    except RuntimeError:
        _dump_forward(raster_settings, inputs)
        raise


def _check_device(t):
    if t.device.type != "cuda":
        raise RuntimeError("the rasterizer runs on the GPU only (no CPU fallback); got tensors on " + str(t.device))
    return t.device


def _fwd_inputs(means3D, opacities, shs, colors_precomp, language_feature, scales, rotations, cov3D_precomp):
    device = _check_device(means3D)
    P = means3D.shape[0]
    means3D = _f32(means3D, device)
    opacities = _f32(opacities, device)
    shs = _opt(shs)
    colors_precomp = _opt(colors_precomp)
    language_feature = _opt(language_feature)
    scales, rotations, cov3D_precomp = _opt(scales), _opt(rotations), _opt(cov3D_precomp)
    shs = _f32(shs, device) if shs is not None else None
    colors_precomp = _f32(colors_precomp, device) if colors_precomp is not None else None
    language_feature = _f32(language_feature, device).reshape(P, -1) if language_feature is not None else None
    scales = _f32(scales, device) if scales is not None else None
    rotations = _f32(rotations, device) if rotations is not None else None
    cov3D_precomp = _f32(cov3D_precomp, device) if cov3D_precomp is not None else None
    M = shs.reshape(P, -1, 3).shape[1] if shs is not None else 0
    C = language_feature.shape[1] if language_feature is not None else 0
    fin = _lib.FwdIn()
    fin.P, fin.M, fin.C = P, M, C
    fin.means3D, fin.shs, fin.colors_precomp = means3D.data_ptr(), _ptr(shs), _ptr(colors_precomp)
    fin.language_feature, fin.opacities = _ptr(language_feature), opacities.data_ptr()
    fin.scales, fin.rotations, fin.cov3D_precomp = _ptr(scales), _ptr(rotations), _ptr(cov3D_precomp)
    inputs = dict(means3D=means3D, opacities=opacities, shs=shs, colors_precomp=colors_precomp,
                  language_feature=language_feature, scales=scales, rotations=rotations, cov3D_precomp=cov3D_precomp)
    return fin, inputs, P


def preprocess_native(raster_settings, means3D, opacities, shs=None, colors_precomp=None, language_feature=None,
                      scales=None, rotations=None, cov3D_precomp=None, stream=None, binning=False,
                      defer_count=False):
    device = _check_device(means3D)
    L = _lib.load()
    stream = stream or torch.cuda.current_stream(device)
    st = _NativeSettings(raster_settings, device)
    fin, inputs, P = _fwd_inputs(means3D, opacities, shs, colors_precomp, language_feature, scales, rotations,
                                 cov3D_precomp)
    H, W = int(raster_settings.image_height), int(raster_settings.image_width)
    with torch.cuda.stream(stream):
        radii = torch.empty(P, dtype=torch.int32, device=device)
        geom = torch.empty(int(L.lsr_geom_bytes(P)), dtype=torch.uint8, device=device)
    fout = _lib.FwdOut()
    fout.radii = radii.data_ptr()
    if defer_count:
        count = torch.zeros(2, dtype=torch.int32, pin_memory=True)
        _check_forward(L.lsr_forward_preprocess_async(ctypes.byref(st.c), ctypes.byref(fin), ctypes.byref(fout),
                                                      ctypes.c_void_p(geom.data_ptr()),
                                                      ctypes.c_void_p(count.data_ptr()),
                                                      ctypes.c_void_p(stream.cuda_stream)),
                       "lsr_forward_preprocess_async", raster_settings, inputs)
        pf = PendingForward(raster_settings, st, fin, inputs, geom, radii, None, device, H, W)
        pf.count_host, pf.stream = count, stream
        pf.counted = torch.cuda.Event()
        pf.counted.record(stream)
        return pf
    K = ctypes.c_int64(0)
    _check_forward(L.lsr_forward_preprocess(ctypes.byref(st.c), ctypes.byref(fin), ctypes.byref(fout),
                                            ctypes.c_void_p(geom.data_ptr()), ctypes.byref(K),
                                            ctypes.c_void_p(stream.cuda_stream)),
                   "lsr_forward_preprocess", raster_settings, inputs)
    pf = PendingForward(raster_settings, st, fin, inputs, geom, radii, K.value, device, H, W)
    if binning:
        _run_binning(pf, stream)
    return pf


def _run_binning(pf, stream):
    L = _lib.load()
    device, H, W, K = pf.device, pf.H, pf.W, pf.num_rendered
    if _BINNING_DELAY_CYCLES:
        with torch.cuda.stream(stream):
            torch.cuda._sleep(_BINNING_DELAY_CYCLES)
    with torch.cuda.stream(stream):
        pf.binning = torch.empty(int(L.lsr_binning_bytes(K)), dtype=torch.uint8, device=device)
        pf.img = torch.empty(int(L.lsr_img_bytes(W, H)), dtype=torch.uint8, device=device)
    _check_forward(L.lsr_forward_binning(ctypes.byref(pf.settings.c), ctypes.byref(pf.fin),
                                         ctypes.c_void_p(pf.geom.data_ptr()), ctypes.c_void_p(pf.binning.data_ptr()),
                                         ctypes.c_void_p(pf.img.data_ptr()), ctypes.c_int64(K),
                                         ctypes.c_void_p(stream.cuda_stream)),
                   "lsr_forward_binning", pf.raster_settings, pf.inputs)
    pf.ready = torch.cuda.Event()
    pf.ready.record(stream)
    pf.ready_stream = stream


def language_split_native(language_feature, stream=None, out=None):
    L = _lib.load()
    device = _check_device(language_feature)
    P, C = language_feature.shape
    stream = stream or torch.cuda.current_stream(device)
    lang = language_feature.detach().to(torch.float32).contiguous()
    if out is None:
        with torch.cuda.stream(stream):
            out = torch.empty(P, 2 * C, dtype=torch.int16, device=device)
    elif out.shape != (P, 2 * C) or out.dtype != torch.int16 or not out.is_contiguous():
        raise ValueError("language_split_native: out must be a contiguous [P, 2C] int16 tensor")
    _lib.check(L.lsr_language_split(P, C, ctypes.c_void_p(lang.data_ptr()), ctypes.c_void_p(out.data_ptr()),
                                    ctypes.c_void_p(stream.cuda_stream)), "lsr_language_split")
    return out


def preprocess_views_native(raster_settings_list, means3D, opacities, shs=None, colors_precomp=None,
                            language_feature=None, scales=None, rotations=None, cov3D_precomp=None, stream=None,
                            split_language=True, split_behind_counts=True, split_stream=None, order_first=None,
                            order_stream=None, row_chunks=None, tile_bucket=False):
    device = _check_device(means3D)
    L = _lib.load()
    stream = stream or torch.cuda.current_stream(device)
    fin, inputs, P = _fwd_inputs(means3D, opacities, shs, colors_precomp, language_feature, scales, rotations,
                                 cov3D_precomp)
    if row_chunks:
        covered = 0
        for r0, r1, _ in row_chunks:
            if r0 != covered or r1 < r0 or r0 % 256:
                raise ValueError("row_chunks must cover [0, P) in order, each r0 a multiple of 256")
            covered = r1
        if covered != P:
            raise ValueError("row_chunks must cover [0, P) in order, each r0 a multiple of 256")
    split = split_language and fin.C == 32 and P > 0
    if split:
        with torch.cuda.stream(stream):
            inputs["language_feature_split"] = torch.empty(P, 64, dtype=torch.int16, device=device)
        fin.language_feature_split = inputs["language_feature_split"].data_ptr()
        if not split_behind_counts and not row_chunks:
            language_split_native(inputs["language_feature"], stream=stream, out=inputs["language_feature_split"])
            split = False
    n = len(raster_settings_list)
    sts = [_NativeSettings(rs, device) for rs in raster_settings_list]
    with torch.cuda.stream(stream):
        radii = [torch.empty(P, dtype=torch.int32, device=device) for _ in range(n)]
        geoms = [torch.empty(int(L.lsr_geom_bytes(P)), dtype=torch.uint8, device=device) for _ in range(n)]
    fouts = [_lib.FwdOut() for _ in range(n)]
    for fo, r in zip(fouts, radii):
        fo.radii = r.data_ptr()
    k = n if (order_first is None or order_stream is None) else max(0, min(int(order_first), n))
    counts = torch.zeros(k, 2, dtype=torch.int32, pin_memory=True) if k > 0 else None
    s_arr, o_arr, g_arr = _settings_array(sts), _struct_array(_lib.FwdOut, fouts), _ptr_array(geoms)
    fi, stp = ctypes.byref(fin), ctypes.c_void_p(stream.cuda_stream)

    def check(rc, what):
        _check_forward(rc, what, raster_settings_list[0], inputs)

    count_fn, count_what = ((L.lsr_forward_instance_scan_views_async, "lsr_forward_instance_scan_views_async")
                            if tile_bucket else
                            (L.lsr_forward_depth_order_views_async, "lsr_forward_depth_order_views_async"))
    if tile_bucket or row_chunks:
        rows_fn, rows_what = ((L.lsr_forward_preprocess_views_tb_async, "lsr_forward_preprocess_views_tb_async")
                              if tile_bucket else
                              (L.lsr_forward_preprocess_views_rows_async, "lsr_forward_preprocess_views_rows_async"))
        for r0, r1, before in (row_chunks or [(0, P, None)]):
            if before is not None:
                before()
            check(rows_fn(n, int(r0), int(r1), s_arr, fi, o_arr, g_arr, stp), rows_what)
        if k > 0:
            check(count_fn(k, s_arr, fi, g_arr, ctypes.c_void_p(counts.data_ptr()), stp), count_what)
    else:
        check(L.lsr_forward_preprocess_views_split_async(n, k, s_arr, fi, o_arr, g_arr,
                                                         ctypes.c_void_p(counts.data_ptr() if k else 0), stp),
              "lsr_forward_preprocess_views_split_async")
    ev = torch.cuda.Event()
    ev.record(stream)
    late = None
    if k < n:
        order_stream.wait_event(ev)
        for g in geoms[k:]:
            g.record_stream(order_stream)
        counts_b = torch.zeros(n - k, 2, dtype=torch.int32, pin_memory=True)
        check(count_fn(n - k, _settings_array(sts[k:]), fi, _ptr_array(geoms[k:]), ctypes.c_void_p(counts_b.data_ptr()),
                       ctypes.c_void_p(order_stream.cuda_stream)), count_what)
        ev_b = torch.cuda.Event()
        ev_b.record(order_stream)
        late = (counts_b, ev_b)
    if split and split_stream is not None:
        split_stream.wait_stream(stream)
        inputs["language_feature_split"].record_stream(split_stream)
        language_split_native(inputs["language_feature"], stream=split_stream, out=inputs["language_feature_split"])
    elif split:
        language_split_native(inputs["language_feature"], stream=stream, out=inputs["language_feature_split"])
    out = []
    for v, rs in enumerate(raster_settings_list):
        H, W = int(rs.image_height), int(rs.image_width)
        pf = PendingForward(rs, sts[v], fin, inputs, geoms[v], radii[v], None, device, H, W)
        pf.tile_bucket = bool(tile_bucket)
        if v < k:
            pf.count_host, pf.stream, pf.counted = counts[v], stream, ev
            pf.count_batch = (counts, v)
        else:
            pf.count_host, pf.stream, pf.counted = late[0][v - k], order_stream, late[1]
            pf.count_batch = (late[0], v - k)
        out.append(pf)
    return out


def _align(nbytes, a=256):
    return (nbytes + a - 1) // a * a


@functools.lru_cache(maxsize=4096)
def _binning_bytes(K):
    return _align(int(_lib.load().lsr_binning_bytes(K)))


@functools.lru_cache(maxsize=4096)
def _binning_bytes_tb(K, P, W, H):
    return _align(int(_lib.load().lsr_binning_bytes_tb(K, P, W, H)))


@functools.lru_cache(maxsize=64)
def _img_bytes(W, H):
    return _align(int(_lib.load().lsr_img_bytes(W, H)))


def _view_arrays(views, *between):
    return (_settings_array([v.settings for v in views]), ctypes.byref(views[0].fin), *between,
            _ptr_array([v.geom for v in views]), _ptr_array([v.binning for v in views]),
            _ptr_array([v.img for v in views]), _int64_array([v.num_rendered for v in views]))


def _forward_outputs(pf):
    H, W, C = pf.H, pf.W, pf.fin.C
    color = torch.empty(3, H, W, dtype=torch.float32, device=pf.device)
    lang_out = torch.empty(C, H, W, dtype=torch.float32, device=pf.device)
    depth = torch.empty(1, H, W, dtype=torch.float32, device=pf.device)
    fout = _lib.FwdOut()
    fout.out_color, fout.out_language_feature = color.data_ptr(), _ptr(lang_out) if C > 0 else None
    fout.radii, fout.out_depth = pf.radii.data_ptr(), depth.data_ptr()
    return color, lang_out, depth, fout


def _wait_for_binning(pf, stream, waited=None):
    if pf.ready_stream is None or pf.ready_stream == stream:
        return
    if waited is None:
        waited = getattr(pf.ready, "_lsr_waited_by", None)
        if waited is None:
            waited = set()
            try:
                pf.ready._lsr_waited_by = waited
            except AttributeError:
                pass
    key = (id(pf.ready), stream.cuda_stream)
    if key not in waited:
        stream.wait_event(pf.ready)
        waited.add(key)


def binning_views_native(pendings, stream=None):
    if not pendings:
        return
    L = _lib.load()
    stream = stream or pendings[0].stream
    batch = pendings[0].count_batch
    if batch is not None and all(pf.count_batch is not None and pf.count_batch[0] is batch[0] for pf in pendings):
        pendings[0].counted.synchronize()
        rows = batch[0].tolist()
        for pf in pendings:
            pf.num_rendered, pf.counted = rows[pf.count_batch[1]][0], None
    else:
        for pf in pendings:
            pf.resolve()
    n = len(pendings)
    device = pendings[0].device
    tb = pendings[0].tile_bucket
    if any(pf.tile_bucket != tb for pf in pendings):
        raise ValueError("binning_views_native: a batch mixes tile-bucket and sort-path views")
    sizes = []
    for pf in pendings:
        sizes += [_binning_bytes_tb(pf.num_rendered, pf.fin.P, pf.W, pf.H) if tb else _binning_bytes(pf.num_rendered),
                  _img_bytes(pf.W, pf.H)]
    with torch.cuda.stream(stream):
        ws = torch.empty(sum(sizes), dtype=torch.uint8, device=device)
    off = 0
    for i, pf in enumerate(pendings):
        pf.binning = ws[off:off + sizes[2 * i]]
        off += sizes[2 * i]
        pf.img = ws[off:off + sizes[2 * i + 1]]
        off += sizes[2 * i + 1]
    fn, what = ((L.lsr_forward_binning_views_tb, "lsr_forward_binning_views_tb") if tb
                else (L.lsr_forward_binning_views, "lsr_forward_binning_views"))
    _check_forward(fn(n, *_view_arrays(pendings), ctypes.c_void_p(stream.cuda_stream)), what,
                   pendings[0].raster_settings, pendings[0].inputs)
    ev = torch.cuda.Event()
    ev.record(stream)
    for pf in pendings:
        pf.ready, pf.ready_stream = ev, stream


def render_native(pending: PendingForward):
    L = _lib.load()
    if pending.tile_bucket and pending.binning is None:
        binning_views_native([pending], stream=torch.cuda.current_stream(pending.device))
    pending.resolve()
    device, H, W = pending.device, pending.H, pending.W
    stream = torch.cuda.current_stream(device)
    pending.geom.record_stream(stream)
    pending.radii.record_stream(stream)
    color, lang_out, depth, fout = _forward_outputs(pending)
    K = pending.num_rendered
    binned = pending.binning is not None
    if binned:
        binning, img = pending.binning, pending.img
        _wait_for_binning(pending, stream)
        binning.record_stream(stream)
        img.record_stream(stream)
    else:
        binning = torch.empty(int(L.lsr_binning_bytes(K)), dtype=torch.uint8, device=device)
        img = torch.empty(int(L.lsr_img_bytes(W, H)), dtype=torch.uint8, device=device)
    fn, what = (L.lsr_forward_composite, "lsr_forward_composite") if binned else (L.lsr_forward_render,
                                                                                   "lsr_forward_render")
    _check_forward(fn(ctypes.byref(pending.settings.c), ctypes.byref(pending.fin), ctypes.byref(fout),
                      ctypes.c_void_p(pending.geom.data_ptr()), ctypes.c_void_p(binning.data_ptr()),
                      ctypes.c_void_p(img.data_ptr()), ctypes.c_int64(K), _stream(device)), what,
# ... 397 lines not shown
```

4dlangsplat_amd/diff_gaussian_rasterization/_lib.py:

```python
from __future__ import annotations

import ctypes
import os

_PKG = os.path.dirname(os.path.dirname(os.path.abspath(__file__)))
LIB_PATH = os.environ.get("LSR_LIBRARY", os.path.join(_PKG, "build", "liblsr.so"))

c_float_p = ctypes.c_void_p
API_VERSION = 4
DEFORM_API_VERSION = 3
QUERY_API_VERSION = 1


class Settings(ctypes.Structure):
    _fields_ = [
        ("image_height", ctypes.c_int32), ("image_width", ctypes.c_int32),
        ("tanfovx", ctypes.c_float), ("tanfovy", ctypes.c_float),
        ("bg", ctypes.c_void_p), ("scale_modifier", ctypes.c_float),
        ("viewmatrix", ctypes.c_void_p), ("projmatrix", ctypes.c_void_p),
        ("sh_degree", ctypes.c_int32), ("campos", ctypes.c_void_p),
        ("prefiltered", ctypes.c_int32), ("debug", ctypes.c_int32), ("include_feature", ctypes.c_int32),
    ]


class FwdIn(ctypes.Structure):
    _fields_ = [
        ("P", ctypes.c_int32), ("M", ctypes.c_int32), ("C", ctypes.c_int32),
        ("means3D", ctypes.c_void_p), ("shs", ctypes.c_void_p), ("colors_precomp", ctypes.c_void_p),
        ("language_feature", ctypes.c_void_p), ("opacities", ctypes.c_void_p), ("scales", ctypes.c_void_p),
        ("rotations", ctypes.c_void_p), ("cov3D_precomp", ctypes.c_void_p),
        ("language_feature_split", ctypes.c_void_p),
    ]


class FwdOut(ctypes.Structure):
    _fields_ = [("out_color", ctypes.c_void_p), ("out_language_feature", ctypes.c_void_p),
                ("radii", ctypes.c_void_p), ("out_depth", ctypes.c_void_p)]


class BwdIn(ctypes.Structure):
    _fields_ = [("dL_dout_color", ctypes.c_void_p), ("dL_dout_language_feature", ctypes.c_void_p),
                ("dL_dout_depth", ctypes.c_void_p), ("deterministic", ctypes.c_int32)]


class BwdOut(ctypes.Structure):
    _fields_ = [("dL_dmeans3D", ctypes.c_void_p), ("dL_dmeans2D", ctypes.c_void_p), ("dL_dcolors", ctypes.c_void_p),
                ("dL_dlanguage_feature", ctypes.c_void_p), ("dL_dopacity", ctypes.c_void_p),
                ("dL_dcov3D", ctypes.c_void_p), ("dL_dsh", ctypes.c_void_p), ("dL_dscales", ctypes.c_void_p),
                ("dL_drotations", ctypes.c_void_p)]


class DeformNet(ctypes.Structure):
    _fields_ = [("n_scales", ctypes.c_int32), ("channels", ctypes.c_int32), ("width", ctypes.c_int32),
                ("res", ctypes.c_int32 * 4), ("multires", ctypes.c_int32 * 4), ("depth", ctypes.c_int32),
                ("heads", ctypes.c_uint32), ("apply_rotation", ctypes.c_int32), ("lang_mode", ctypes.c_int32),
                ("lang_dim", ctypes.c_int32), ("centers", ctypes.c_int32), ("time_pe", ctypes.c_int32),
                ("aabb", ctypes.c_void_p), ("planes", (ctypes.c_void_p * 6) * 4),
                ("w_feat", ctypes.c_void_p * 4), ("b_feat", ctypes.c_void_p * 4),
                ("w1", ctypes.c_void_p * 6), ("b1", ctypes.c_void_p * 6), ("w2", ctypes.c_void_p * 6),
                ("b2", ctypes.c_void_p * 6), ("w_lang", ctypes.c_void_p * 3), ("b_lang", ctypes.c_void_p * 3)]


class DeformGrads(ctypes.Structure):
    _fields_ = [("planes", (ctypes.c_void_p * 6) * 4), ("w_feat", ctypes.c_void_p * 4), ("b_feat", ctypes.c_void_p * 4),
                ("w1", ctypes.c_void_p * 6), ("b1", ctypes.c_void_p * 6), ("w2", ctypes.c_void_p * 6),
                ("b2", ctypes.c_void_p * 6), ("w_lang", ctypes.c_void_p * 3), ("b_lang", ctypes.c_void_p * 3),
                ("aabb", ctypes.c_void_p)]


class AdamGroup(ctypes.Structure):
    _fields_ = [("param", ctypes.c_void_p), ("grad", ctypes.c_void_p), ("exp_avg", ctypes.c_void_p),
                ("exp_avg_sq", ctypes.c_void_p), ("n", ctypes.c_int64), ("lr", ctypes.c_double),
                ("step", ctypes.c_int64)]


class RowTensor(ctypes.Structure):
    _fields_ = [("src", ctypes.c_void_p), ("dst", ctypes.c_void_p), ("row_bytes", ctypes.c_int64),
                ("zero_from", ctypes.c_int64)]


class SegView(ctypes.Structure):
    _fields_ = [("image", ctypes.c_void_p), ("d_image", ctypes.c_void_p), ("seg", ctypes.c_void_p),
                ("table", ctypes.c_void_p), ("n_seg", ctypes.c_int32)]


class Decoder(ctypes.Structure):
    _fields_ = [("n_layers", ctypes.c_int32), ("dims", ctypes.c_int32 * 9), ("weight", ctypes.c_void_p * 8),
                ("bias", ctypes.c_void_p * 8)]


ADAM_MAX_GROUPS = 16
GATHER_MAX_TENSORS = 32
SEG_LOSS_MAX_VIEWS = 8
QUERY_MAX_LAYERS = 8
QUERY_MAX_PHRASES = 64
QUERY_MAX_WIDTH = 512
QUERY_MAX_INPUT = 32
SEGMENT_MAX_SCALE = 63
SEGMENT_MAX_SIDE = 16384
SEGMENT_STRATEGIES = {"point": 0, "mean": 1}

_vp = ctypes.c_void_p
SIGNATURES = {
    "lsr_adam_step": (ctypes.c_int, [ctypes.POINTER(AdamGroup), ctypes.c_int32, ctypes.c_double, ctypes.c_double,
                                     ctypes.c_double, _vp]),
    "lsr_densify_stats": (ctypes.c_int, [ctypes.c_int32, _vp, _vp, ctypes.c_int32, _vp, _vp, _vp, _vp]),
    "lsr_train_workspace_bytes": (ctypes.c_int64, [ctypes.c_int32]),
    "lsr_densify_plan": (ctypes.c_int, [ctypes.c_int32, _vp, _vp, _vp, ctypes.c_float, ctypes.c_float, ctypes.c_float,
                                        ctypes.c_int32, _vp, _vp, _vp, _vp]),
    "lsr_prune_plan": (ctypes.c_int, [ctypes.c_int32, _vp, _vp, _vp, ctypes.c_float, ctypes.c_float, ctypes.c_float,
                                      _vp, _vp, _vp, _vp]),
    "lsr_gather_rows": (ctypes.c_int, [ctypes.c_int32, ctypes.POINTER(RowTensor), _vp, ctypes.c_int64, _vp]),
    "lsr_split_fixup": (ctypes.c_int, [ctypes.c_int64, ctypes.c_int64, ctypes.c_int32, _vp, _vp, _vp, _vp, _vp, _vp,
                                       _vp, _vp]),
    "lsr_reset_opacity": (ctypes.c_int, [ctypes.c_int32, _vp, _vp, _vp, _vp]),
    "lsr_activate": (ctypes.c_int, [ctypes.c_int32] + [_vp] * 7),
    "lsr_l1_workspace_bytes": (ctypes.c_int64, [ctypes.c_int32]),
    "lsr_l1_loss_views": (ctypes.c_int, [ctypes.c_int32, ctypes.c_int64, _vp, _vp, ctypes.c_int64, _vp, _vp, _vp]),
    "lsr_l1_loss_views_backward": (ctypes.c_int, [ctypes.c_int32, ctypes.c_int64, _vp, _vp, ctypes.c_int64, _vp, _vp,
                                                  _vp]),
    "lsr_seg_loss_workspace_bytes": (ctypes.c_int64, [ctypes.c_int32] * 4),
    "lsr_seg_loss_views": (ctypes.c_int, [ctypes.c_int32] * 4 + [ctypes.POINTER(SegView), ctypes.c_float,
                                          ctypes.c_float, ctypes.c_int32, _vp, _vp, _vp]),
    "lsr_seg_loss_views_backward": (ctypes.c_int, [ctypes.c_int32] * 4 + [ctypes.POINTER(SegView), ctypes.c_float,
                                                   ctypes.c_float, ctypes.c_int32, _vp, _vp, _vp]),
    "lsr_repeat_rows": (ctypes.c_int, [ctypes.c_int32, ctypes.POINTER(RowTensor), ctypes.c_int64, ctypes.c_int32, _vp]),
    "lsr_sum_row_blocks": (ctypes.c_int, [ctypes.c_int32, ctypes.POINTER(RowTensor), ctypes.c_int64, ctypes.c_int32,
                                          _vp]),
    "lsr_activate_backward": (ctypes.c_int, [ctypes.c_int32] + [_vp] * 10),
    "lsr_version": (ctypes.c_int, []),
    "lsr_require_api": (ctypes.c_int, [ctypes.c_int32]),
    "lsr_deform_require_api": (ctypes.c_int, [ctypes.c_int32]),
    "lsr_last_error": (ctypes.c_char_p, []),
    "lsr_geom_bytes": (ctypes.c_int64, [ctypes.c_int32]),
    "lsr_binning_bytes": (ctypes.c_int64, [ctypes.c_int64]),
    "lsr_img_bytes": (ctypes.c_int64, [ctypes.c_int32, ctypes.c_int32]),
    "lsr_backward_bytes": (ctypes.c_int64, [ctypes.c_int32, ctypes.c_int64, ctypes.c_int32, ctypes.c_int32]),
    "lsr_forward_preprocess": (ctypes.c_int, [ctypes.POINTER(Settings), ctypes.POINTER(FwdIn), ctypes.POINTER(FwdOut),
                                              ctypes.c_void_p, ctypes.POINTER(ctypes.c_int64), ctypes.c_void_p]),
    "lsr_forward_preprocess_async": (ctypes.c_int, [ctypes.POINTER(Settings), ctypes.POINTER(FwdIn),
                                                    ctypes.POINTER(FwdOut), ctypes.c_void_p, ctypes.c_void_p,
                                                    ctypes.c_void_p]),
    "lsr_forward_preprocess_views_async": (ctypes.c_int, [ctypes.c_int32, ctypes.POINTER(ctypes.POINTER(Settings)),
                                                          ctypes.POINTER(FwdIn), ctypes.POINTER(ctypes.POINTER(FwdOut)),
                                                          ctypes.POINTER(ctypes.c_void_p), ctypes.c_void_p,
                                                          ctypes.c_void_p]),
    "lsr_forward_preprocess_views_split_async": (ctypes.c_int, [ctypes.c_int32, ctypes.c_int32,
                                                                ctypes.POINTER(ctypes.POINTER(Settings)),
                                                                ctypes.POINTER(FwdIn),
                                                                ctypes.POINTER(ctypes.POINTER(FwdOut)),
                                                                ctypes.POINTER(ctypes.c_void_p), ctypes.c_void_p,
                                                                ctypes.c_void_p]),
    "lsr_forward_preprocess_views_rows_async": (ctypes.c_int, [ctypes.c_int32, ctypes.c_int32, ctypes.c_int32,
                                                               ctypes.POINTER(ctypes.POINTER(Settings)),
                                                               ctypes.POINTER(FwdIn),
                                                               ctypes.POINTER(ctypes.POINTER(FwdOut)),
                                                               ctypes.POINTER(ctypes.c_void_p), ctypes.c_void_p]),
    "lsr_forward_depth_order_views_async": (ctypes.c_int, [ctypes.c_int32, ctypes.POINTER(ctypes.POINTER(Settings)),
                                                           ctypes.POINTER(FwdIn), ctypes.POINTER(ctypes.c_void_p),
                                                           ctypes.c_void_p, ctypes.c_void_p]),
    "lsr_forward_binning_views": (ctypes.c_int, [ctypes.c_int32, ctypes.POINTER(ctypes.POINTER(Settings)),
                                                 ctypes.POINTER(FwdIn), ctypes.POINTER(ctypes.c_void_p),
                                                 ctypes.POINTER(ctypes.c_void_p), ctypes.POINTER(ctypes.c_void_p),
                                                 ctypes.POINTER(ctypes.c_int64), ctypes.c_void_p]),
    "lsr_binning_bytes_tb": (ctypes.c_int64, [ctypes.c_int64, ctypes.c_int32, ctypes.c_int32, ctypes.c_int32]),
    "lsr_forward_preprocess_views_tb_async": (ctypes.c_int, [ctypes.c_int32, ctypes.c_int32, ctypes.c_int32,
                                                             ctypes.POINTER(ctypes.POINTER(Settings)),
                                                             ctypes.POINTER(FwdIn),
                                                             ctypes.POINTER(ctypes.POINTER(FwdOut)),
                                                             ctypes.POINTER(ctypes.c_void_p), ctypes.c_void_p]),
    "lsr_forward_instance_scan_views_async": (ctypes.c_int, [ctypes.c_int32, ctypes.POINTER(ctypes.POINTER(Settings)),
                                                             ctypes.POINTER(FwdIn), ctypes.POINTER(ctypes.c_void_p),
                                                             ctypes.c_void_p, ctypes.c_void_p]),
    "lsr_forward_binning_views_tb": (ctypes.c_int, [ctypes.c_int32, ctypes.POINTER(ctypes.POINTER(Settings)),
                                                    ctypes.POINTER(FwdIn), ctypes.POINTER(ctypes.c_void_p),
                                                    ctypes.POINTER(ctypes.c_void_p), ctypes.POINTER(ctypes.c_void_p),
                                                    ctypes.POINTER(ctypes.c_int64), ctypes.c_void_p]),
    "lsr_forward_render": (ctypes.c_int, [ctypes.POINTER(Settings), ctypes.POINTER(FwdIn), ctypes.POINTER(FwdOut),
                                          ctypes.c_void_p, ctypes.c_void_p, ctypes.c_void_p, ctypes.c_int64,
                                          ctypes.c_void_p]),
    "lsr_forward_binning": (ctypes.c_int, [ctypes.POINTER(Settings), ctypes.POINTER(FwdIn), ctypes.c_void_p,
                                           ctypes.c_void_p, ctypes.c_void_p, ctypes.c_int64, ctypes.c_void_p]),
    "lsr_forward_composite": (ctypes.c_int, [ctypes.POINTER(Settings), ctypes.POINTER(FwdIn), ctypes.POINTER(FwdOut),
                                             ctypes.c_void_p, ctypes.c_void_p, ctypes.c_void_p, ctypes.c_int64,
                                             ctypes.c_void_p]),
    "lsr_forward_composite_views": (ctypes.c_int, [ctypes.c_int32, ctypes.POINTER(ctypes.POINTER(Settings)),
                                                   ctypes.POINTER(FwdIn), ctypes.POINTER(ctypes.POINTER(FwdOut)),
                                                   ctypes.POINTER(ctypes.c_void_p), ctypes.POINTER(ctypes.c_void_p),
                                                   ctypes.POINTER(ctypes.c_void_p), ctypes.POINTER(ctypes.c_int64),
                                                   ctypes.c_void_p]),
    "lsr_backward_composite_views": (ctypes.c_int, [ctypes.c_int32, ctypes.POINTER(ctypes.POINTER(Settings)),
                                                    ctypes.POINTER(FwdIn), ctypes.POINTER(ctypes.POINTER(BwdIn)),
                                                    ctypes.c_void_p, ctypes.POINTER(ctypes.c_void_p),
                                                    ctypes.POINTER(ctypes.c_void_p), ctypes.POINTER(ctypes.c_void_p),
                                                    ctypes.POINTER(ctypes.c_int64), ctypes.c_void_p]),
    "lsr_backward": (ctypes.c_int, [ctypes.POINTER(Settings), ctypes.POINTER(FwdIn), ctypes.POINTER(BwdIn),
                                    ctypes.POINTER(BwdOut), ctypes.c_void_p, ctypes.c_void_p, ctypes.c_void_p,
                                    ctypes.c_void_p, ctypes.c_int64, ctypes.c_int32, ctypes.c_void_p]),
    "lsr_backward_views": (ctypes.c_int, [ctypes.c_int32, ctypes.POINTER(ctypes.POINTER(Settings)), ctypes.POINTER(FwdIn),
                                          ctypes.POINTER(ctypes.POINTER(BwdIn)), ctypes.POINTER(BwdOut),
                                          ctypes.POINTER(ctypes.c_void_p), ctypes.POINTER(ctypes.c_void_p),
                                          ctypes.POINTER(ctypes.c_void_p), ctypes.POINTER(ctypes.c_int64),
                                          ctypes.c_int32, ctypes.c_void_p]),
    "lsr_backward_composite": (ctypes.c_int, [ctypes.POINTER(Settings), ctypes.POINTER(FwdIn), ctypes.POINTER(BwdIn),
                                              ctypes.c_void_p, ctypes.c_void_p, ctypes.c_void_p, ctypes.c_void_p,
                                              ctypes.c_int64, ctypes.c_void_p]),
    "lsr_backward_preprocess_views": (ctypes.c_int, [ctypes.c_int32, ctypes.POINTER(ctypes.POINTER(Settings)),
                                                     ctypes.POINTER(FwdIn), ctypes.POINTER(BwdOut),
                                                     ctypes.POINTER(ctypes.c_void_p), ctypes.c_int32, ctypes.c_void_p]),
    "lsr_backward_preprocess_views_rows": (ctypes.c_int, [ctypes.c_int32, ctypes.POINTER(ctypes.POINTER(Settings)),
                                                          ctypes.POINTER(FwdIn), ctypes.POINTER(BwdOut),
                                                          ctypes.POINTER(ctypes.c_void_p), ctypes.c_int32,
                                                          ctypes.c_int32, ctypes.c_int32, ctypes.c_void_p]),
    "lsr_language_split": (ctypes.c_int, [ctypes.c_int32, ctypes.c_int32, ctypes.c_void_p, ctypes.c_void_p,
                                          ctypes.c_void_p]),
    "lsr_radii_max": (ctypes.c_int, [ctypes.c_int32, ctypes.c_int32, ctypes.POINTER(ctypes.c_void_p), ctypes.c_void_p,
                                     ctypes.c_int32, ctypes.c_void_p]),
    "lsr_mark_visible": (ctypes.c_int, [ctypes.c_int32, ctypes.c_void_p, ctypes.c_void_p, ctypes.c_void_p,
                                        ctypes.c_void_p, ctypes.c_void_p]),
    "lsr_profile_enable": (ctypes.c_int, [ctypes.c_int32]),
    "lsr_profile_phases": (ctypes.c_int, [ctypes.c_uint32]),
    "lsr_knn_workspace_bytes": (ctypes.c_int64, [ctypes.c_int32]),
    "lsr_knn_mean_dist": (ctypes.c_int, [ctypes.c_int32, ctypes.c_void_p, ctypes.c_void_p, ctypes.c_void_p,
                                         ctypes.c_void_p]),
    "lsr_deform_workspace_bytes": (ctypes.c_int64, [ctypes.POINTER(DeformNet)]),
    "lsr_deform_prepare": (ctypes.c_int, [ctypes.POINTER(DeformNet), ctypes.c_void_p, ctypes.c_void_p]),
    "lsr_deform_forward": (ctypes.c_int, [ctypes.POINTER(DeformNet), ctypes.c_void_p, ctypes.c_int32]
                           + [ctypes.c_void_p] * 14 + [ctypes.c_void_p]),
    "lsr_deform_backward_scratch_bytes": (ctypes.c_int64, [ctypes.POINTER(DeformNet), ctypes.c_int32]),
    "lsr_deform_backward": (ctypes.c_int, [ctypes.POINTER(DeformNet), ctypes.c_void_p, ctypes.c_int32]
                            + [ctypes.c_void_p] * 14 + [ctypes.POINTER(DeformGrads), ctypes.c_void_p, ctypes.c_void_p]),
    "lsr_query_require_api": (ctypes.c_int, [ctypes.c_int32]),
    "lsr_query_relevancy": (ctypes.c_int, [ctypes.POINTER(Decoder), ctypes.c_int64, _vp, ctypes.c_int64, ctypes.c_int64,
                                           ctypes.c_int32, _vp, ctypes.c_int32, _vp, ctypes.c_float, _vp, _vp]),
    "lsr_query_decode": (ctypes.c_int, [ctypes.POINTER(Decoder), ctypes.c_int64, _vp, ctypes.c_int64, ctypes.c_int64,
                                        _vp, _vp]),
    "lsr_segment_workspace_bytes": (ctypes.c_int64, [ctypes.c_int32] * 3),
    "lsr_segment": (ctypes.c_int, [ctypes.c_int32] * 3 + [_vp, ctypes.c_int32, ctypes.c_float, ctypes.c_int32, _vp,
                                   ctypes.c_int32] + [_vp] * 8),
    "lsr_profile_read": (ctypes.c_int, [ctypes.POINTER(ctypes.c_double), ctypes.POINTER(ctypes.c_int64),
                                        ctypes.c_int32]),
}

PHASES = ["preprocess", "depth_sort", "instance_scan", "emit", "tile_sort", "tile_ranges", "render_fwd",
          "render_bwd", "preprocess_bwd", "preprocess_bwd_views"]


def profile_enable(on=True, phases=None):
    L = load()
    L.lsr_profile_phases(0xFFFFFFFF if phases is None else sum(1 << PHASES.index(p) for p in phases))
    L.lsr_profile_enable(1 if on else 0)


def profile_read():
    n = len(PHASES)
    ms = (ctypes.c_double * n)()
    cnt = (ctypes.c_int64 * n)()
    load().lsr_profile_read(ms, cnt, n)
    return {PHASES[i]: (ms[i], cnt[i]) for i in range(n)}

_LIB = None


def load():
    global _LIB
    if _LIB is None:
        path = os.environ.get("LSR_LIBRARY", LIB_PATH)
        if not os.path.exists(path):
            raise ImportError(f"liblsr.so not found at {LIB_PATH}; build it with `make -C 4dlangsplat_amd/csrc` "
                              "(or __graft_entry__.build()).  There is no CPU fallback.")
        lib = ctypes.CDLL(path)
        for name, (res, args) in SIGNATURES.items():
            fn = getattr(lib, name)
            fn.restype = res
            fn.argtypes = args
        if (lib.lsr_require_api(API_VERSION) != 0 or lib.lsr_deform_require_api(DEFORM_API_VERSION) != 0
                or lib.lsr_query_require_api(QUERY_API_VERSION) != 0):
            raise ImportError(f"{path}: {lib.lsr_last_error().decode()} (rebuild it: make -C 4dlangsplat_amd/csrc)")
        _LIB = lib
    return _LIB


def check(rc: int, what: str):
    if rc != 0:
        msg = load().lsr_last_error()
        raise RuntimeError(f"{what} failed (code {rc}): {msg.decode() if msg else ''}")
```

4dlangsplat_amd/view_parallel.py:

```python
import os
from typing import Callable, Dict, Optional, Tuple

import torch
import torch.distributed as dist

GRAD_FIELDS = (("means3D", 3), ("scales", 3), ("rotations", 4), ("opacities", 1), ("sh", None),
               ("language_feature", None))


def _free_port() -> int:
    import socket
    with socket.socket() as s:
        s.bind(("127.0.0.1", 0))
        return s.getsockname()[1]


def _rank_child(rank: int, fn: Callable, world: int, fn_args: tuple):
    os.environ.update(RANK=str(rank), LOCAL_RANK=str(rank), WORLD_SIZE=str(world),
                      LOCAL_WORLD_SIZE=str(world))
    fn(rank, world, *fn_args)


def launch_ranks(world: int, fn: Callable, fn_args: tuple = ()) -> None:
    import torch.multiprocessing as mp
# ... 30 lines not shown
        self.ranges: Dict[str, Tuple[int, int]] = {}
        o = 0
        for name, w in fields:
            seg = self.flat[o * Pa:o * Pa + w * P]
            self.ranges[name] = (o * Pa, (o + w) * Pa)
            if w == 0:
                self.views[name] = None
            elif name == "sh":
                self.views[name] = seg.view(P, M, 3)
            else:
                self.views[name] = seg.view(P, w)
            o += w
        self.radii = torch.zeros(P, dtype=torch.int32, device=device) if densify_stats else None

    def zero_(self):
        self.flat.zero_()
        if self.radii is not None:
            self.radii.zero_()

    def zero_accumulated_(self):
        lo, hi = self.ranges["language_feature"]
        if hi > lo:
            self.flat[lo:hi].zero_()
        if self.radii is not None:
            self.radii.zero_()

    def need(self) -> Dict[str, bool]:
        return dict(means3D=True, scales=True, rotations=True, opacities=True, sh=self.M > 0,
                    language_feature=self.C > 0, means2D=self.densify_stats, colors=False, cov3D=False)

    @property
    def nbytes(self) -> int:
        return self.flat.numel() * 4


def row_chunks(P: int, n: int, align: int = 256):
    if P <= 0:
        return [(0, 0)]
    step = -(-P // max(1, n))
    step = -(-step // align) * align
    return [(r0, min(P, r0 + step)) for r0 in range(0, P, step)]


class ViewParallelStep:

    def __init__(self, bucket: GradBucket, n_views: int, group=None, flush_chunks: int = 4, update=None,
                 defer_gather: bool = False):
        self.update = update
        self.defer_gather = bool(defer_gather)
        self.bucket = bucket
        self.n_views = n_views
        self.group = group
        self.flush_chunks = flush_chunks
        self.distributed = dist.is_available() and dist.is_initialized()
        self.world = dist.get_world_size(group) if self.distributed else 1
        self.rank = dist.get_rank(group) if self.distributed else 0
        self.views = range(*view_slice(n_views, self.world, self.rank))

    def run(self, render_view: Callable[[int, GradBucket], Optional[torch.Tensor]]) -> GradBucket:
        b = self.bucket
        upd = self.update
        defer = False
        if upd is not None and hasattr(upd, "gather_waits"):
            waits = upd.gather_waits()
            setter = getattr(render_view, "set_row_waits", None) if self.defer_gather else None
            if waits and setter is not None:
                setter(waits)
                upd._ag = []
            else:
                upd.wait_all()
            defer = setter is not None
        begin = getattr(render_view, "begin_step", None)
        if begin is not None:
            begin(self.views)
        flush = getattr(render_view, "flush", None)
        zero = b.zero_accumulated_ if getattr(flush, "overwrites", False) else b.zero_
        batch = getattr(render_view, "render_batch", None)
        if batch is not None:
            if getattr(batch, "before_wait", False):
                radii_views = [r for r in batch(self.views, b, before_wait=zero) if r is not None]
            else:
                zero()
                radii_views = [r for r in batch(self.views, b) if r is not None]
            if b.radii is None:
                radii_views = []
        else:
            zero()
            radii_views = []
            for v in self.views:
                radii = render_view(v, b)
                if b.radii is not None and radii is not None:
                    radii_views.append(radii)
        if not (batch is not None and getattr(batch, "radii_reduced", False)):
            for radii in radii_views:
                torch.maximum(b.radii, radii.to(torch.int32), out=b.radii)
        pending = []
        lo, hi = b.ranges["language_feature"]
        if self.world > 1 and b.radii is not None:
            pending.append(dist.all_reduce(b.radii, op=dist.ReduceOp.MAX, group=self.group, async_op=True))
        sharded = self.update is not None
        if self.world > 1 and flush is not None and hi > lo and not sharded:
            pending.append(dist.all_reduce(b.flat[lo:hi], op=dist.ReduceOp.SUM, group=self.group, async_op=True))
        chunked = self.world > 1 and getattr(flush, "chunked", False) and self.flush_chunks > 1 and not sharded
        sharded_chunks = sharded and getattr(flush, "chunked", False) and getattr(self.update, "chunks", 1) > 1
        if sharded_chunks:
            flush(b, row_chunks=self.update.chunk_rows(), on_rows=lambda r0, r1: self.update.on_rows(b, r0, r1))
        elif chunked:
            def on_rows(r0, r1):
                for name, (f0, f1) in b.ranges.items():
                    w = b.widths[name]
                    if name == "language_feature" or w == 0 or r1 <= r0:
                        continue
                    pending.append(dist.all_reduce(b.flat[f0 + r0 * w:f0 + r1 * w], op=dist.ReduceOp.SUM,
                                                   group=self.group, async_op=True))
            flush(b, row_chunks=row_chunks(b.P, self.flush_chunks), on_rows=on_rows)
        elif flush is not None:
            flush(b)
        end = getattr(render_view, "end_step", None)
        if end is not None:
            end()
        if sharded:
            if defer:
                self.update.step(b, wait_gather=False)
            else:
                self.update.step(b)
            for h in pending:
                h.wait()
        elif self.world > 1:
            if not chunked:
                if flush is not None and hi > lo:
                    segs = (b.flat[:lo], b.flat[hi:])
                else:
                    segs = (b.flat,)
                for seg in segs:
                    if seg.numel():
                        dist.all_reduce(seg, op=dist.ReduceOp.SUM, group=self.group)
            for h in pending:
                h.wait()
        return b

    def finish(self) -> None:
        if self.update is not None and hasattr(self.update, "wait_all"):
            self.update.wait_all()

    def visibility(self) -> torch.Tensor:
        if self.bucket.radii is None:
            raise RuntimeError("visibility needs GradBucket(densify_stats=True)")
        return self.bucket.radii > 0


def native_view_renderer(scene, settings, grad_fn: Callable, deterministic: bool = False, overlap: bool = True,
                         batch_backward: bool = True, early_views=3, composite_batch: bool = True,
                         side_priority: int = 0, side_from_preprocess: bool = True, split_behind_counts: bool = True,
                         fill_on_side: bool = False, order_on_side: bool = False, tile_bucket: bool = False):
    import diff_gaussian_rasterization as dgr

    lookahead = overlap == "lookahead"
    batch_fwd = overlap == "batched"
    side = (torch.cuda.Stream(device=scene.means3D.device) if (overlap and not lookahead and not batch_fwd)
            else None)
    bin_side = [None]
    pending = {}
    fill_ready = [None]
    params_ready = torch.cuda.Event() if side is not None else None
    step_views = [None]

    def has_view(v):
        if step_views[0] is not None and v not in step_views[0]:
            return False
        return v in settings if isinstance(settings, dict) else 0 <= v < len(settings)

    def preprocess(v, stream=None, defer=False):
        return dgr.preprocess_native(settings[v], scene.means3D, scene.opacities, shs=scene.shs,
                                     language_feature=scene.lang, scales=scene.scales, rotations=scene.rotations,
                                     stream=stream, binning=stream is not None, defer_count=defer)

    batched = batch_backward and not deterministic
    held = []
    row_waits = [None]

    def take_row_waits(chunked_ok):
        w, row_waits[0] = row_waits[0], None
        if not w or chunked_ok:
            return w
        for _, _, fn in w:
            fn()
        return None

    def batch_preprocess(v, before_wait=None, radii_out=None):
        views = [w for w in step_views[0] if w >= v] if step_views[0] is not None else [v]
        views = [w for w in views if has_view(w)] or [v]
        sizes = tuple(early_views) if isinstance(early_views, (tuple, list)) else (early_views,)
        e0 = int(sizes[0])
        split_side = 0 < e0 < len(views) and scene.means3D.is_cuda
        if split_side and bin_side[0] is None:
            bin_side[0] = torch.cuda.Stream(device=scene.means3D.device, priority=side_priority)
        to_side = fill_on_side and split_side
        late_order = order_on_side and split_side and not to_side
        waits = take_row_waits(scene.means3D.is_cuda)
        pfs = dgr.preprocess_views_native([settings[w] for w in views], scene.means3D, scene.opacities,
                                          shs=scene.shs, language_feature=scene.lang, scales=scene.scales,
                                          rotations=scene.rotations, split_behind_counts=split_behind_counts,
                                          split_stream=bin_side[0] if to_side else None,
                                          order_first=e0 if late_order else None,
                                          order_stream=bin_side[0] if late_order else None,
                                          row_chunks=waits, tile_bucket=tile_bucket)
        fill_ready[0] = None
        if to_side:
            bin_side[0].wait_stream(torch.cuda.current_stream(scene.means3D.device))
            with torch.cuda.stream(bin_side[0]):
                if before_wait is not None:
                    before_wait()
                if radii_out is not None:
                    for pf in pfs:
                        pf.radii.record_stream(bin_side[0])
                    dgr.radii_max_native([pf.radii for pf in pfs], radii_out, stream=bin_side[0])
            fill_ready[0] = torch.cuda.Event()
            fill_ready[0].record(bin_side[0])
        else:
            if before_wait is not None:
                before_wait()
            if radii_out is not None:
                dgr.radii_max_native([pf.radii for pf in pfs], radii_out)
        if late_order:
            dgr.binning_views_native(pfs[:e0])
        elif split_side:
            dev = scene.means3D.device
            side_b = bin_side[0]
            if side_from_preprocess and not to_side:
                side_b.wait_stream(torch.cuda.current_stream(dev))
            dgr.binning_views_native(pfs[:e0])
            if not side_from_preprocess:
                side_b.wait_stream(torch.cuda.current_stream(dev))
            for pf in pfs[e0:]:
                pf.geom.record_stream(side_b)
            cuts = [e0]
            for n in sizes[1:]:
                if cuts[-1] + int(n) < len(views):
                    cuts.append(cuts[-1] + int(n))
            cuts.append(len(views))
            for a0, a1 in zip(cuts, cuts[1:]):
                dgr.binning_views_native(pfs[a0:a1], stream=side_b)
        else:
            dgr.binning_views_native(pfs)
        pending.update(zip(views, pfs))

    def render_view(v: int, bucket: GradBucket):
        if batch_fwd and v not in pending:
            batch_preprocess(v)
        take_row_waits(False)
        pf = pending.pop(v, None)
        if pf is None:
            pf = preprocess(v)
            if params_ready is not None:
                params_ready.record(torch.cuda.current_stream())
        if lookahead:
            pf.resolve(binning=True)
            if has_view(v + 1):
                pending[v + 1] = preprocess(v + 1, defer=True)
        color, lang, radii, depth, st = dgr.render_native(pf)
        gc, gl, gd = grad_fn(v, color, lang, depth)
        if batched:
            held.append(dgr.backward_composite_native(st, gc, gl, gd, dL_dlanguage=bucket.views["language_feature"]))
        else:
            dgr.backward_native(st, gc, gl, gd, out=bucket.views, accumulate=True, need=bucket.need(),
                                deterministic=deterministic)
        render_view.last_num_rendered = st.num_rendered
        if side is not None and has_view(v + 1):
            side.wait_event(params_ready)
            pending[v + 1] = preprocess(v + 1, stream=side)
        return radii

    def render_batch(views, bucket: GradBucket, before_wait=None):
        views = list(views)
        if not views:
            if before_wait is not None:
                before_wait()
            return []
        reduce_radii = bucket.radii is not None and scene.means3D.is_cuda
        fresh = views[0] not in pending
        if fresh:
            batch_preprocess(views[0], before_wait, radii_out=bucket.radii if reduce_radii else None)
        elif before_wait is not None:
            before_wait()
        pfs = [pending.pop(v) for v in views]
        if fill_ready[0] is not None:
            torch.cuda.current_stream(scene.means3D.device).wait_event(fill_ready[0])
            fill_ready[0] = None
        groups = []
        for v, pf in zip(views, pfs):
            if groups and groups[-1][0][1].ready is pf.ready:
                groups[-1].append((v, pf))
            else:
                groups.append([(v, pf)])
        radii, ks = [], []
        sizes = tuple(early_views) if isinstance(early_views, (tuple, list)) else (early_views,)
        split_groups = []
        for grp in groups:
            unbinned = [pf for _, pf in grp if getattr(pf, "binning", True) is None]
            if unbinned and unbinned[0].stream is not None and unbinned[0].stream != torch.cuda.current_stream(
                    scene.means3D.device):
                cuts = [0]
                for n in sizes[1:]:
                    if cuts[-1] + int(n) < len(grp):
                        cuts.append(cuts[-1] + int(n))
                cuts.append(len(grp))
                for a0, a1 in zip(cuts, cuts[1:]):
                    dgr.binning_views_native([pf for _, pf in grp[a0:a1]], stream=unbinned[0].stream)
                    split_groups.append(grp[a0:a1])
            else:
                split_groups.append(grp)
        for grp in split_groups:
            res = dgr.render_views_native([pf for _, pf in grp])
            gcs, gls, gds = [], [], []
            for (v, _), (color, lang, r, depth, st) in zip(grp, res):
                gc, gl, gd = grad_fn(v, color, lang, depth)
                gcs.append(gc)
                gls.append(gl)
                gds.append(gd)
                radii.append(r)
                ks.append(st.num_rendered)
            held.extend(dgr.backward_composite_views_native([x[4] for x in res], gcs, gls, gds,
                                                            dL_dlanguage=bucket.views["language_feature"]))
        if reduce_radii and not fresh:
            dgr.radii_max_native(radii, bucket.radii)
        render_batch.last_num_rendered = ks
        render_batch.radii_reduced = reduce_radii
        return radii

    def flush(bucket: GradBucket, row_chunks=None, on_rows=None):
        if held:
            dgr.backward_preprocess_views_native(held, out=bucket.views, accumulate=False, need=bucket.need(),
                                                 row_chunks=row_chunks, on_rows=on_rows)
            held.clear()
        else:
            lo, hi = bucket.ranges["language_feature"]
            bucket.flat[:lo].zero_()
            bucket.flat[hi:].zero_()
            for r0, r1 in (row_chunks or []):
                if on_rows is not None:
                    on_rows(r0, r1)

    flush.overwrites = True
    flush.chunked = True

    def begin_step(views):
        pending.clear()
        step_views[0] = range(views.start, views.stop) if isinstance(views, range) else list(views)

    def end_step():
        pending.clear()
        step_views[0] = None

    def set_row_waits(waits):
        row_waits[0] = list(waits) if waits else None

    render_view.begin_step = begin_step
    render_view.end_step = end_step
    render_view.set_row_waits = set_row_waits
    render_view.pending = pending
    render_view.last_num_rendered = 0
    if batched:
        render_view.flush = flush
        if batch_fwd and composite_batch:
            render_batch.last_num_rendered = []
            render_batch.before_wait = True
            render_view.render_batch = render_batch
    return render_view


class ShardedAdam:

    GROUPS = ("xyz", "f_dc", "f_rest", "opacity", "scaling", "rotation", "language_feature")
    BUCKET_FIELDS = ("means3D", "scales", "rotations", "opacities", "sh", "language_feature")
    ACT_FIELDS = ("means3D", "scales", "rotations", "opacities", "shs", "lang")

    @staticmethod
    def row_multiple(P: int, world: int, align: int = 64, chunks: int = 1) -> int:
        align = max(align, 256) if chunks > 1 else align
        unit = world * max(1, chunks) * align
        return -(-max(P, 1) // unit) * unit

    def __init__(self, scene, raw: Dict[str, torch.Tensor], lrs: Dict[str, float], group=None, align: int = 64,
                 betas=(0.9, 0.999), eps: float = 1e-15, adam: Optional[Callable] = None, nonormalized: bool = False,
                 chunks: int = 1):
        if getattr(scene, "deformation", None) is not None:
            raise ValueError("ShardedAdam steps the rasterizer inputs directly: a scene with a deformation "
                             "field needs the field's backward between the bucket and the parameters")
        self.distributed = dist.is_available() and dist.is_initialized()
        self.group = group
        self.world = dist.get_world_size(group) if self.distributed else 1
        self.rank = dist.get_rank(group) if self.distributed else 0
        self.xyz_scheduler_args = None
        self.chunks = max(1, int(chunks))
        self.P = P = scene.means3D.shape[0]
        self.Pa = self.row_multiple(P, self.world, align, self.chunks) if P > 0 else 0
        self.Pc = self.Pa // self.chunks
        self.piece = self.Pc // self.world
        self.rows = self.chunks * self.piece
        self.pieces = [(c * self.Pc + self.rank * self.piece, c * self.Pc + (self.rank + 1) * self.piece)
                       for c in range(self.chunks)]
        self.r0 = min(P, self.pieces[0][0]) if self.pieces else 0
        self.r1 = min(P, self.pieces[0][1]) if self.pieces else 0
        self.lrs, self.betas, self.eps, self.nonormalized = dict(lrs), betas, eps, nonormalized
        self._adam = adam
        self.scene = scene
        dev = scene.means3D.device
        self.act = {}
        for name in self.ACT_FIELDS:
            t = getattr(scene, name)
            buf = torch.zeros((self.Pa,) + tuple(t.shape[1:]), dtype=torch.float32, device=dev)
            buf[:P] = t
            self.act[name] = buf
            setattr(scene, name, buf[:P])
        self.raw = {}
        for n in self.GROUPS:
            if n not in raw:
                continue
            src = raw[n].detach().to(dev, torch.float32)
            t = torch.zeros((self.rows,) + tuple(src.shape[1:]), dtype=torch.float32, device=dev)
            for c, (g0, g1) in enumerate(self.pieces):
                hi = min(g1, P)
                if hi > g0:
                    t[c * self.piece:c * self.piece + hi - g0] = src[g0:hi]
            self.raw[n] = t.contiguous()
        self.exp_avg = {n: torch.zeros_like(t) for n, t in self.raw.items()}
        self.exp_avg_sq = {n: torch.zeros_like(t) for n, t in self.raw.items()}
        self.steps = {n: 0 for n in self.raw}
        self._rs = {}
        self._ag = []
        self.grad_hook: Optional[Callable] = None

    def set_xyz_schedule(self, lr_init, lr_final, lr_delay_mult=0.01, max_steps=30000):
        from gaussian_train import get_expon_lr_func
        self.xyz_scheduler_args = get_expon_lr_func(lr_init=lr_init, lr_final=lr_final, lr_delay_mult=lr_delay_mult,
# ... 159 lines not shown
```

include/lsr.h:

```cpp
#ifndef LSR_H_
#define LSR_H_

#include <stddef.h>
#include <stdint.h>

#ifdef __cplusplus
extern "C" {
#endif

#define LSR_API_VERSION 4

#define LSR_OK 0
#define LSR_EINVAL 1
#define LSR_EHIP 2
#define LSR_ECAPACITY 3

typedef void *lsr_stream_t;

typedef struct lsr_settings {
    int32_t image_height;
    int32_t image_width;
    float tanfovx;
    float tanfovy;
    const float *bg;
    float scale_modifier;
    const float *viewmatrix;
    const float *projmatrix;
    int32_t sh_degree;
    const float *campos;
    int32_t prefiltered;
    int32_t debug;
    int32_t include_feature;
} lsr_settings;

typedef struct lsr_fwd_in {
    int32_t P;
    int32_t M;
    int32_t C;
    const float *means3D;
    const float *shs;
    const float *colors_precomp;
    const float *language_feature;
    const float *opacities;
    const float *scales;
    const float *rotations;
    const float *cov3D_precomp;
    const uint16_t *language_feature_split;
} lsr_fwd_in;

typedef struct lsr_fwd_out {
    float *out_color;
    float *out_language_feature;
    int32_t *radii;
    float *out_depth;
} lsr_fwd_out;

typedef struct lsr_bwd_in {
    const float *dL_dout_color;
    const float *dL_dout_language_feature;
    const float *dL_dout_depth;
    int32_t deterministic;
} lsr_bwd_in;

typedef struct lsr_bwd_out {
    float *dL_dmeans3D;
    float *dL_dmeans2D;
    float *dL_dcolors;
    float *dL_dlanguage_feature;
    float *dL_dopacity;
    float *dL_dcov3D;
    float *dL_dsh;
    float *dL_dscales;
    float *dL_drotations;
} lsr_bwd_out;

int lsr_version(void);
const char *lsr_last_error(void);
int lsr_require_api(int32_t caller_version);

int64_t lsr_geom_bytes(int32_t P);
int64_t lsr_binning_bytes(int64_t num_rendered);
int64_t lsr_img_bytes(int32_t image_width, int32_t image_height);
int64_t lsr_backward_bytes(int32_t P, int64_t num_rendered, int32_t C, int32_t deterministic);

int lsr_forward_preprocess(const lsr_settings *s, const lsr_fwd_in *in, lsr_fwd_out *out, void *geom,
                           int64_t *num_rendered, lsr_stream_t stream);

int lsr_forward_preprocess_async(const lsr_settings *s, const lsr_fwd_in *in, lsr_fwd_out *out, void *geom,
                                 uint32_t *host_count, lsr_stream_t stream);

int lsr_forward_preprocess_views_async(int32_t n_views, const lsr_settings *const *s, const lsr_fwd_in *in,
                                       lsr_fwd_out *const *out, void *const *geom, uint32_t *host_counts,
                                       lsr_stream_t stream);

int lsr_forward_preprocess_views_split_async(int32_t n_views, int32_t n_ordered, const lsr_settings *const *s,
                                             const lsr_fwd_in *in, lsr_fwd_out *const *out, void *const *geom,
                                             uint32_t *host_counts, lsr_stream_t stream);
int lsr_forward_preprocess_views_rows_async(int32_t n_views, int32_t row0, int32_t row1, const lsr_settings *const *s,
                                            const lsr_fwd_in *in, lsr_fwd_out *const *out, void *const *geom,
                                            lsr_stream_t stream);
int lsr_forward_depth_order_views_async(int32_t n_views, const lsr_settings *const *s, const lsr_fwd_in *in,
                                        void *const *geom, uint32_t *host_counts, lsr_stream_t stream);

int lsr_forward_render(const lsr_settings *s, const lsr_fwd_in *in, lsr_fwd_out *out, void *geom,
                       void *binning, void *img, int64_t num_rendered, lsr_stream_t stream);

int lsr_forward_binning(const lsr_settings *s, const lsr_fwd_in *in, void *geom, void *binning, void *img,
                        int64_t num_rendered, lsr_stream_t stream);
int lsr_forward_composite(const lsr_settings *s, const lsr_fwd_in *in, lsr_fwd_out *out, const void *geom,
                          const void *binning, void *img, int64_t num_rendered, lsr_stream_t stream);
int lsr_forward_binning_views(int32_t n_views, const lsr_settings *const *s, const lsr_fwd_in *in,
                              void *const *geom, void *const *binning, void *const *img,
                              const int64_t *num_rendered, lsr_stream_t stream);

int64_t lsr_binning_bytes_tb(int64_t num_rendered, int32_t P, int32_t image_width, int32_t image_height);
int lsr_forward_preprocess_views_tb_async(int32_t n_views, int32_t row0, int32_t row1, const lsr_settings *const *s,
                                          const lsr_fwd_in *in, lsr_fwd_out *const *out, void *const *geom,
                                          lsr_stream_t stream);
int lsr_forward_instance_scan_views_async(int32_t n_views, const lsr_settings *const *s, const lsr_fwd_in *in,
                                          void *const *geom, uint32_t *host_counts, lsr_stream_t stream);
int lsr_forward_binning_views_tb(int32_t n_views, const lsr_settings *const *s, const lsr_fwd_in *in,
                                 void *const *geom, void *const *binning, void *const *img,
                                 const int64_t *num_rendered, lsr_stream_t stream);
int lsr_forward_composite_views(int32_t n_views, const lsr_settings *const *s, const lsr_fwd_in *in,
                                lsr_fwd_out *const *out, const void *const *geom, const void *const *binning,
                                void *const *img, const int64_t *num_rendered, lsr_stream_t stream);

int lsr_backward(const lsr_settings *s, const lsr_fwd_in *in, const lsr_bwd_in *gin, lsr_bwd_out *gout,
                 const void *geom, const void *binning, const void *img, void *scratch, int64_t num_rendered,
                 int32_t accumulate, lsr_stream_t stream);

int lsr_backward_views(int32_t n_views, const lsr_settings *const *s, const lsr_fwd_in *in,
                       const lsr_bwd_in *const *gin, lsr_bwd_out *gout, void *const *geom,
                       const void *const *binning, const void *const *img, const int64_t *num_rendered,
                       int32_t accumulate, lsr_stream_t stream);

int lsr_backward_composite(const lsr_settings *s, const lsr_fwd_in *in, const lsr_bwd_in *gin, float *dL_dlanguage,
                           void *geom, const void *binning, const void *img, int64_t num_rendered,
                           lsr_stream_t stream);
int lsr_backward_composite_views(int32_t n_views, const lsr_settings *const *s, const lsr_fwd_in *in,
                                 const lsr_bwd_in *const *gin, float *dL_dlanguage, void *const *geom,
                                 const void *const *binning, const void *const *img,
                                 const int64_t *num_rendered, lsr_stream_t stream);
int lsr_backward_preprocess_views(int32_t n_views, const lsr_settings *const *s, const lsr_fwd_in *in,
                                  lsr_bwd_out *gout, const void *const *geom, int32_t accumulate,
                                  lsr_stream_t stream);
int lsr_backward_preprocess_views_rows(int32_t n_views, const lsr_settings *const *s, const lsr_fwd_in *in,
                                       lsr_bwd_out *gout, const void *const *geom, int32_t accumulate,
                                       int32_t row_begin, int32_t row_count, lsr_stream_t stream);

int lsr_language_split(int32_t P, int32_t C, const float *language_feature, uint16_t *out, lsr_stream_t stream);

int lsr_radii_max(int32_t P, int32_t n_views, const int32_t *const *radii, int32_t *out, int32_t accumulate,
                  lsr_stream_t stream);

int lsr_mark_visible(int32_t P, const float *means3D, const float *viewmatrix, const float *projmatrix,
                     uint8_t *present, lsr_stream_t stream);

#define LSR_PHASE_PREPROCESS 0
#define LSR_PHASE_DEPTH_SORT 1
#define LSR_PHASE_INSTANCE_SCAN 2
#define LSR_PHASE_EMIT 3
#define LSR_PHASE_TILE_SORT 4
#define LSR_PHASE_TILE_RANGES 5
#define LSR_PHASE_RENDER_FWD 6
#define LSR_PHASE_RENDER_BWD 7
#define LSR_PHASE_PREPROCESS_BWD 8
#define LSR_PHASE_PREPROCESS_BWD_VIEWS 9
#define LSR_NUM_PHASES 10
int lsr_profile_enable(int32_t on);
int lsr_profile_phases(uint32_t mask);
int lsr_profile_read(double *ms_total, int64_t *launches, int32_t n);

#ifdef __cplusplus
}
#endif
#endif
```

Before: 975.4 frames/s.

## Fuse language split, grad zeroing and radii max into multi-view preprocess

Adds an optional fused preprocess entry point. In one kernel pass it converts language features to split bf16, zeroes the gradient accumulator rows and reduces the per-Gaussian max radius across views, replacing separate launches. Separately, preprocess no longer writes the identity order array; the depth-sort scatter instead generates the index values in-register via an IOTA template. The preprocess kernel also gets a waves_per_eu hint. This saves several full-P memory passes and launches, at the cost of more register pressure and extra per-wave work inside preprocess. The fused path only runs when the Python caller passes `fused_preprocess=True`.

```diff
diff --git a/4dlangsplat_amd/csrc/lsr_api.hip b/4dlangsplat_amd/csrc/lsr_api.hip
--- a/4dlangsplat_amd/csrc/lsr_api.hip
+++ b/4dlangsplat_amd/csrc/lsr_api.hip
@@ -308,7 +308,7 @@
     v.view = s->viewmatrix; v.proj = s->projmatrix; v.campos = s->campos;
     v.radii = radii; v.radius = g.radius; v.tiles = g.tiles; v.rect = g.rect; v.key = g.key_a; v.xy = g.xy;
     v.conic_o = g.conic_o; v.rgbd = g.rgbd; v.clamped = g.clamped;
-    v.order = g.val_a;
+    v.order = nullptr;
     v.rank_counts = g.counts;
     v.acc = g.acc;
     v.clear.p[0] = g.total;
@@ -406,11 +406,13 @@
 }
 
 int preprocess_rows(int32_t n_views, int32_t row0, int32_t row1, int counts_tiles, const lsr_settings* const* s,
-                    const lsr_fwd_in* in, lsr_fwd_out* const* out, void* const* geom, hipStream_t st) {
+                    const lsr_fwd_in* in, lsr_fwd_out* const* out, void* const* geom, const lsr_preprocess_fused* f,
+                    hipStream_t st) {
     const int P = in->P;
     if (row1 == row0) return LSR_OK;
     for (int v0 = 0; v0 < n_views; v0 += lsr::LSR_MAX_VIEWS) {
         const int nv = std::min(n_views - v0, lsr::LSR_MAX_VIEWS);
+        const bool first = v0 == 0;
         lsr::PreprocessArgs a{};
         preprocess_shared(a, s[v0], in);
         a.nv = nv;
@@ -420,12 +422,59 @@
         for (int k = 0; k < nv; ++k) {
             Geom g = carve_geom(geom[v0 + k], (size_t)P, nullptr);
             preprocess_view(a.v[k], s[v0 + k], g, out[v0 + k]->radii);
+            if (counts_tiles) a.v[k].order = g.val_a;
+        }
+        if (f && nv > 1) {
+            if (first && f->language_split_out) {
+                a.lang = in->language_feature;
+                a.lang_split_out = f->language_split_out;
+            }
+            if (first && f->zero_rows) {
+                a.zero_rows_out = f->zero_rows;
+                a.zero_row_floats = f->zero_row_floats;
+            }
+            a.radii_max_out = f->radii_max_out;
+            a.radii_max_accumulate = (f->radii_max_accumulate || !first) ? 1 : 0;
         }
         {
             PhaseTimer t(LSR_PHASE_PREPROCESS, st);
             lsr::launch_preprocess(a, st);
         }
         LSR_LAUNCHED("preprocess", st, s[v0]->debug);
+        if (f && nv == 1) {
+            const int n = row1 - row0;
+            if (first && f->language_split_out)
+                lsr::launch_language_split(n, in->language_feature + (size_t)row0 * 32,
+                                           f->language_split_out + (size_t)row0 * 64, st);
+            if (first && f->zero_rows)
+                LSR_HIP(hipMemsetAsync(f->zero_rows + (size_t)row0 * f->zero_row_floats, 0,
+                                       (size_t)n * f->zero_row_floats * sizeof(float), st));
+            if (f->radii_max_out) {
+                const int* r = out[v0]->radii + row0;
+                lsr::launch_radii_max(n, 1, &r, f->radii_max_out + row0, f->radii_max_accumulate || !first, st);
+            }
+            LSR_LAUNCHED("preprocess per-step outputs", st, s[v0]->debug);
+        }
+    }
+    return LSR_OK;
+}
+
+int check_fused(const lsr_preprocess_fused* f, int32_t n_views, const lsr_fwd_in* in, lsr_fwd_out* const* out) {
+    if (!f) return LSR_OK;
+    if (f->language_split_out) {
+        if (in->C != 32 || (in->P > 0 && !in->language_feature))
+            return fail(LSR_EINVAL, "fused preprocess: the language split needs C == 32 and the language rows");
+        if ((size_t)in->P * 32 * 4 >= (size_t)1 << 32)
+            return fail(LSR_EINVAL, "fused preprocess: P * C * 4 must be < 2^32");
+        if ((reinterpret_cast<uintptr_t>(f->language_split_out) | reinterpret_cast<uintptr_t>(in->language_feature)) & 15)
+            return fail(LSR_EINVAL, "fused preprocess: the language rows and the split buffer must be 16-byte aligned");
+    }
+    if ((f->zero_rows != nullptr) != (f->zero_row_floats > 0) || f->zero_row_floats < 0)
+        return fail(LSR_EINVAL, "fused preprocess: zero_rows and a positive zero_row_floats go together");
+    if (f->radii_max_out) {
+        uintptr_t al = reinterpret_cast<uintptr_t>(f->radii_max_out);
+        if (n_views % lsr::LSR_MAX_VIEWS == 1 && out && out[n_views - 1]) al |= reinterpret_cast<uintptr_t>(out[n_views - 1]->radii);
+        if (al & 15) return fail(LSR_EINVAL, "fused preprocess: radii_max_out and the radii arrays must be 16-byte aligned");
     }
     return LSR_OK;
 }
@@ -441,6 +490,7 @@
             ss[k] = lsr::SortSeg{g.key_a, g.val_a, g.key_b, g.val_b, g.sort_tmp, g.total + 3,
                                  lsr::SortGather{g.rect, g.counts, g.rect_sorted}, (size_t)P};
             ss[k].vals_c = g.offsets;
+            ss[k].iota_vals = 1;
         }
         {
             PhaseTimer t(LSR_PHASE_DEPTH_SORT, st);
@@ -470,24 +520,27 @@
 namespace {
 int preprocess_and_order(int32_t n_views, int32_t n_ordered, const lsr_settings* const* s, const lsr_fwd_in* in,
                          lsr_fwd_out* const* out, void* const* geom, uint32_t* host_counts, bool map_counts,
-                         hipStream_t st) {
+                         const lsr_preprocess_fused* fused, hipStream_t st) {
     if (in->P == 0) {
         for (int v = 0; v < 2 * n_ordered; ++v) host_counts[v] = 0;
         return LSR_OK;
     }
-    int rc = preprocess_rows(n_views, 0, in->P, 0, s, in, out, geom, st);
+    int rc = preprocess_rows(n_views, 0, in->P, 0, s, in, out, geom, fused, st);
     if (rc || n_ordered == 0) return rc;
     return depth_order_views(n_ordered, s, in, geom, host_counts, map_counts ? mapped_counts(host_counts) : nullptr, st);
 }
 
 int preprocess_rows_checked(int32_t n_views, int32_t row0, int32_t row1, int counts_tiles, const lsr_settings* const* s,
-                            const lsr_fwd_in* in, lsr_fwd_out* const* out, void* const* geom, lsr_stream_t stream) {
+                            const lsr_fwd_in* in, lsr_fwd_out* const* out, void* const* geom,
+                            const lsr_preprocess_fused* fused, lsr_stream_t stream) {
     int rc = check_views(n_views, s, in, geom);
     if (rc) return rc;
     if (!out || row0 < 0 || row1 < row0 || row1 > in->P || row0 % 256 != 0)
         return fail(LSR_EINVAL, "0 <= row0 <= row1 <= P with row0 a multiple of 256, and the outputs are required");
     if ((rc = need_radii(n_views, out, in->P))) return rc;
-    return preprocess_rows(n_views, row0, row1, counts_tiles, s, in, out, geom, reinterpret_cast<hipStream_t>(stream));
+    if ((rc = check_fused(fused, n_views, in, out))) return rc;
+    return preprocess_rows(n_views, row0, row1, counts_tiles, s, in, out, geom, fused,
+                           reinterpret_cast<hipStream_t>(stream));
 }
 
 int count_views(int32_t n_views, const lsr_settings* const* s, const lsr_fwd_in* in, void* const* geom,
@@ -578,31 +631,48 @@
     if (rc) return rc;
     if ((rc = need_radii(1, &out, in->P))) return rc;
     if (!geom || !host_count) return fail(LSR_EINVAL, "geom workspace and host_count are required");
-    return preprocess_and_order(1, 1, &s, in, &out, &geom, host_count, false, reinterpret_cast<hipStream_t>(stream));
+    return preprocess_and_order(1, 1, &s, in, &out, &geom, host_count, false, nullptr,
+                                reinterpret_cast<hipStream_t>(stream));
+}
+
+int lsr_forward_preprocess_views_split_fused_async(int32_t n_views, int32_t n_ordered, const lsr_settings* const* s,
+                                                   const lsr_fwd_in* in, lsr_fwd_out* const* out, void* const* geom,
+                                                   uint32_t* host_counts, const lsr_preprocess_fused* fused,
+                                                   lsr_stream_t stream) {
+    int rc = check_views(n_views, s, in, geom);
+    if (rc) return rc;
+    if (!out || (n_ordered > 0 && !host_counts) || n_ordered < 0 || n_ordered > n_views)
+        return fail(LSR_EINVAL, "0 <= n_ordered <= n_views, the outputs and host_counts are required");
+    if ((rc = need_radii(n_views, out, in->P))) return rc;
+    if ((rc = check_fused(fused, n_views, in, out))) return rc;
+    return preprocess_and_order(n_views, n_ordered, s, in, out, geom, host_counts, true, fused,
+                                reinterpret_cast<hipStream_t>(stream));
 }
 
 int lsr_forward_preprocess_views_split_async(int32_t n_views, int32_t n_ordered, const lsr_settings* const* s,
                                              const lsr_fwd_in* in, lsr_fwd_out* const* out, void* const* geom,
                                              uint32_t* host_counts, lsr_stream_t stream) {
-    int rc = check_views(n_views, s, in, geom);
-    if (rc) return rc;
-    if (!out || (n_ordered > 0 && !host_counts) || n_ordered < 0 || n_ordered > n_views)
-        return fail(LSR_EINVAL, "0 <= n_ordered <= n_views, the outputs and host_counts are required");
-    if ((rc = need_radii(n_views, out, in->P))) return rc;
-    return preprocess_and_order(n_views, n_ordered, s, in, out, geom, host_counts, true,
-                                reinterpret_cast<hipStream_t>(stream));
+    return lsr_forward_preprocess_views_split_fused_async(n_views, n_ordered, s, in, out, geom, host_counts, nullptr,
+                                                          stream);
+}
+
+int lsr_forward_preprocess_views_rows_fused_async(int32_t n_views, int32_t row0, int32_t row1,
+                                                  const lsr_settings* const* s, const lsr_fwd_in* in,
+                                                  lsr_fwd_out* const* out, void* const* geom,
+                                                  const lsr_preprocess_fused* fused, lsr_stream_t stream) {
+    return preprocess_rows_checked(n_views, row0, row1, 0, s, in, out, geom, fused, stream);
 }
 
 int lsr_forward_preprocess_views_rows_async(int32_t n_views, int32_t row0, int32_t row1, const lsr_settings* const* s,
                                             const lsr_fwd_in* in, lsr_fwd_out* const* out, void* const* geom,
                                             lsr_stream_t stream) {
-    return preprocess_rows_checked(n_views, row0, row1, 0, s, in, out, geom, stream);
+    return preprocess_rows_checked(n_views, row0, row1, 0, s, in, out, geom, nullptr, stream);
 }
 
 int lsr_forward_preprocess_views_tb_async(int32_t n_views, int32_t row0, int32_t row1, const lsr_settings* const* s,
                                           const lsr_fwd_in* in, lsr_fwd_out* const* out, void* const* geom,
                                           lsr_stream_t stream) {
-    return preprocess_rows_checked(n_views, row0, row1, 1, s, in, out, geom, stream);
+    return preprocess_rows_checked(n_views, row0, row1, 1, s, in, out, geom, nullptr, stream);
 }
 
 int lsr_forward_instance_scan_views_async(int32_t n_views, const lsr_settings* const* s, const lsr_fwd_in* in,
diff --git a/4dlangsplat_amd/csrc/lsr_internal.h b/4dlangsplat_amd/csrc/lsr_internal.h
--- a/4dlangsplat_amd/csrc/lsr_internal.h
+++ b/4dlangsplat_amd/csrc/lsr_internal.h
@@ -80,6 +80,12 @@
     const float* colors_precomp;
     const float* cov3D_precomp;
     PreprocessView v[LSR_MAX_VIEWS];
+    const float* lang;
+    uint16_t* lang_split_out;
+    float* zero_rows_out;
+    int zero_row_floats;
+    int radii_max_accumulate;
+    int* radii_max_out;
 };
 
 struct ViewCam {
@@ -341,6 +347,7 @@
     uint2* ranges;
     uint32_t nranges;
     uint32_t* vals_c;
+    uint32_t iota_vals;
 };
 struct SortBatch { SortSeg s[LSR_MAX_VIEWS]; };
 int radix_sort_batch(const SortSeg* segs, int nseg, int begin_bit, int end_bit, hipStream_t st);
diff --git a/4dlangsplat_amd/csrc/preprocess.hip b/4dlangsplat_amd/csrc/preprocess.hip
--- a/4dlangsplat_amd/csrc/preprocess.hip
+++ b/4dlangsplat_amd/csrc/preprocess.hip
@@ -1,5 +1,6 @@
 #include "lsr_common.h"
 #include "lsr_internal.h"
+#include "lsr_mfma.h"
 
 namespace lsr {
 
@@ -131,7 +132,8 @@
 
 template <int MS, bool PRE>
 __device__ __forceinline__ bool preprocess_one(const PreprocessArgs& a, const PreprocessView& v, const GaussIn<MS>& g,
-                                               int i) {
+                                               int i, int& radius_out) {
+    radius_out = 0;
     v.radii[i] = 0;
     v.radius[i] = 0;
     v.tiles[i] = 0;
@@ -244,6 +246,7 @@
     }
     v.radii[i] = radius;
     v.radius[i] = radius;
+    radius_out = radius;
     uint32_t qmap = 0;
     if (ntiles > 0 && cmax.x - cmin.x <= 2 && cmax.y - cmin.y <= 2) {
         const EmitSplat es = emit_splat(pix, conic);
@@ -285,22 +288,79 @@
     }
 }
 
+__device__ __forceinline__ void split_lang_rows(const float* __restrict__ lang, uint16_t* __restrict__ out, int row0,
+                                                int P) {
+    const int ln = threadIdx.x & 63;
+    const int rows = min(64, P - row0);
+    if (rows <= 0) return;
+    const float4* src = reinterpret_cast<const float4*>(lang) + (size_t)row0 * 8;
+    bf16x4* dst = reinterpret_cast<bf16x4*>(out) + (size_t)row0 * 16;
+    float4 x[8];
+#pragma unroll
+    for (int q = 0; q < 8; ++q) {
+        const int e = q * 64 + ln;
+        x[q] = e < rows * 8 ? src[e] : make_float4(0.0f, 0.0f, 0.0f, 0.0f);
+    }
+#pragma unroll
+    for (int q = 0; q < 8; ++q) {
+        const int e = q * 64 + ln;
+        const float f[4] = {x[q].x, x[q].y, x[q].z, x[q].w};
+        bf16x4 h, l;
+#pragma unroll
+        for (int j = 0; j < 4; ++j) {
+            __bf16 hh, ll;
+            split_bf16(f[j], hh, ll);
+            h[j] = hh;
+            l[j] = ll;
+        }
+        if (e < rows * 8) {
+            const int r = e >> 3, c4 = e & 7;
+            dst[r * 16 + c4] = h;
+            dst[r * 16 + 8 + c4] = l;
+        }
+    }
+}
+
+__device__ __forceinline__ void zero_rows(float* __restrict__ out, int w, int row0, int P) {
+    const int ln = threadIdx.x & 63;
+    const int rows = min(64, P - row0);
+    if (rows <= 0) return;
+    float* d = out + (size_t)row0 * w;
+    const int n = rows * w;
+    if ((w & 3) == 0 && (reinterpret_cast<uintptr_t>(out) & 15) == 0) {
+        for (int e = ln; e < n / 4; e += 64) reinterpret_cast<float4*>(d)[e] = make_float4(0.0f, 0.0f, 0.0f, 0.0f);
+    } else {
+        for (int e = ln; e < n; e += 64) d[e] = 0.0f;
+    }
+}
+
 template <int MS, bool MULTI>
-__global__ void __launch_bounds__(256) k_preprocess(PreprocessArgs a) {
+__global__ void __launch_bounds__(256) __attribute__((amdgpu_waves_per_eu(3))) k_preprocess(PreprocessArgs a) {
     const int i = a.row0 + blockIdx.x * blockDim.x + threadIdx.x;
     GaussIn<MS> g;
     if constexpr (!MULTI) {
+        int radius;
         clear_words(a.v[0].clear);
-        const bool rect = i < a.P && preprocess_one<MS, false>(a, a.v[0], g, i);
+        const bool rect = i < a.P && preprocess_one<MS, false>(a, a.v[0], g, i, radius);
         zero_acc_rows(a.v[0].acc, rect, i);
     } else {
         const bool ok = i < a.P;
+        const int wrow0 = i - (int)(threadIdx.x & 63);
+        if (a.lang_split_out) split_lang_rows(a.lang, a.lang_split_out, wrow0, a.P);
+        if (a.zero_rows_out) zero_rows(a.zero_rows_out, a.zero_row_floats, wrow0, a.P);
         if (ok) load_gauss<MS>(a, i, g);
+        int rmax = 0;
         for (int k = 0; k < a.nv; ++k) {
             const PreprocessView& v = a.v[k];
             clear_words(v.clear);
-            const bool rect = ok && preprocess_one<MS, true>(a, v, g, i);
+            int radius = 0;
+            const bool rect = ok && preprocess_one<MS, true>(a, v, g, i, radius);
+            rmax = max(rmax, radius);
             zero_acc_rows(v.acc, rect, i);
+        }
+        if (a.radii_max_out && ok) {
+            if (a.radii_max_accumulate) rmax = max(rmax, a.radii_max_out[i]);
+            a.radii_max_out[i] = rmax;
         }
     }
 }
diff --git a/4dlangsplat_amd/csrc/sort.hip b/4dlangsplat_amd/csrc/sort.hip
--- a/4dlangsplat_amd/csrc/sort.hip
+++ b/4dlangsplat_amd/csrc/sort.hip
@@ -447,7 +447,7 @@
 
 constexpr int SCAN_DG = 16;
 
-template <int IT>
+template <int IT, bool IOTA = false>
 __global__ void __launch_bounds__(256) k_rts_scatter(const SortBatch b, int pass, int in_b, int shift, int nbits_h,
                                                      int last_h) {
     __shared__ uint32_t s_key[(256 * IT)];
@@ -489,7 +489,8 @@
         const size_t idx = base + (size_t)r * 64 + lane;
         const bool valid = idx < n;
         key[r] = valid ? keys_in[idx] : 0u;
-        val[r] = valid ? vals_in[idx] : 0u;
+        if constexpr (IOTA) val[r] = (uint32_t)idx;
+        else val[r] = valid ? vals_in[idx] : 0u;
     }
     const int da = 2 * tid, db = 2 * tid + 1;
     const uint32_t pre_a = da < nd ? offs[(size_t)bid * RDX + da] : 0u, pre_b = db < nd ? offs[(size_t)bid * RDX + db] : 0u;
@@ -589,6 +590,9 @@
     if (ns == 0 || end_bit <= begin_bit) return 0;
     for (int i = 1; i < ns; ++i)
         if ((bt.s[i].vals_c == nullptr) != (bt.s[0].vals_c == nullptr)) return -1;
+    const bool iota = bt.s[0].iota_vals != 0;
+    for (int i = 1; i < ns; ++i)
+        if ((bt.s[i].iota_vals != 0) != iota) return -1;
     if (bt.s[0].vals_c && (begin_bit != 0 || end_bit != 32)) return -1;
     for (int i = 0; i < ns; ++i) {
         const SortSeg& g = bt.s[i];
@@ -602,7 +606,14 @@
         else
             hipLaunchKernelGGL(k_rts_count<OS_ITEMS>, dim3(nbi, ns), dim3(256), 0, st, bt, p, in_b, shift, nbits);
         hipLaunchKernelGGL(k_rts_scan<SCAN_DG>, dim3(RDX / SCAN_DG, ns), dim3(256), 0, st, bt, p, items, in_b, nbits);
-        if (items == 12)
+        if (iota && p == 0) {
+            if (items == 12)
+                hipLaunchKernelGGL((k_rts_scatter<12, true>), dim3(nbi, ns), dim3(256), 0, st, bt, p, in_b, shift, nbits,
+                                   last);
+            else
+                hipLaunchKernelGGL((k_rts_scatter<OS_ITEMS, true>), dim3(nbi, ns), dim3(256), 0, st, bt, p, in_b, shift,
+                                   nbits, last);
+        } else if (items == 12)
             hipLaunchKernelGGL(k_rts_scatter<12>, dim3(nbi, ns), dim3(256), 0, st, bt, p, in_b, shift, nbits, last);
         else
             hipLaunchKernelGGL(k_rts_scatter<OS_ITEMS>, dim3(nbi, ns), dim3(256), 0, st, bt, p, in_b, shift, nbits,
diff --git a/4dlangsplat_amd/diff_gaussian_rasterization/__init__.py b/4dlangsplat_amd/diff_gaussian_rasterization/__init__.py
--- a/4dlangsplat_amd/diff_gaussian_rasterization/__init__.py
+++ b/4dlangsplat_amd/diff_gaussian_rasterization/__init__.py
@@ -248,7 +248,8 @@
 def preprocess_views_native(raster_settings_list, means3D, opacities, shs=None, colors_precomp=None,
                             language_feature=None, scales=None, rotations=None, cov3D_precomp=None, stream=None,
                             split_language=True, split_behind_counts=True, split_stream=None, order_first=None,
-                            order_stream=None, row_chunks=None, tile_bucket=False):
+                            order_stream=None, row_chunks=None, tile_bucket=False, fuse_split=False, zero_rows=None,
+                            radii_max_out=None, radii_max_accumulate=False):
     device = _check_device(means3D)
     L = _lib.load()
     stream = stream or torch.cuda.current_stream(device)
@@ -270,6 +271,25 @@
         if not split_behind_counts and not row_chunks:
             language_split_native(inputs["language_feature"], stream=stream, out=inputs["language_feature_split"])
             split = False
+    fused = None
+    if (fuse_split or zero_rows is not None or radii_max_out is not None) and P > 0:
+        if tile_bucket:
+            raise ValueError("preprocess_views_native: the per-step outputs are the sort path's (tile_bucket=False)")
+        fused = _lib.PreprocessFused()
+        if zero_rows is not None:
+            if (zero_rows.dim() != 2 or zero_rows.shape[0] != P or zero_rows.shape[1] < 1 or zero_rows.dtype != torch.float32
+                    or not zero_rows.is_contiguous() or zero_rows.device != device):
+                raise ValueError("preprocess_views_native: zero_rows must be a contiguous float32 [P, w] tensor")
+            fused.zero_rows, fused.zero_row_floats = zero_rows.data_ptr(), int(zero_rows.shape[1])
+        if radii_max_out is not None:
+            if (radii_max_out.shape != (P,) or radii_max_out.dtype != torch.int32 or not radii_max_out.is_contiguous()
+                    or radii_max_out.device != device):
+                raise ValueError("preprocess_views_native: radii_max_out must be a contiguous int32 [P] tensor")
+            fused.radii_max_out, fused.radii_max_accumulate = radii_max_out.data_ptr(), 1 if radii_max_accumulate else 0
+        if fuse_split and split and split_stream is None and inputs["language_feature"].data_ptr() % 16 == 0:
+            fused.language_split_out = inputs["language_feature_split"].data_ptr()
+            split = False
+    fz = ctypes.byref(fused) if fused is not None else None
     n = len(raster_settings_list)
     sts = [_NativeSettings(rs, device) for rs in raster_settings_list]
     with torch.cuda.stream(stream):
@@ -290,19 +310,22 @@
                             if tile_bucket else
                             (L.lsr_forward_depth_order_views_async, "lsr_forward_depth_order_views_async"))
     if tile_bucket or row_chunks:
-        rows_fn, rows_what = ((L.lsr_forward_preprocess_views_tb_async, "lsr_forward_preprocess_views_tb_async")
-                              if tile_bucket else
-                              (L.lsr_forward_preprocess_views_rows_async, "lsr_forward_preprocess_views_rows_async"))
         for r0, r1, before in (row_chunks or [(0, P, None)]):
             if before is not None:
                 before()
-            check(rows_fn(n, int(r0), int(r1), s_arr, fi, o_arr, g_arr, stp), rows_what)
+            if tile_bucket:
+                check(L.lsr_forward_preprocess_views_tb_async(n, int(r0), int(r1), s_arr, fi, o_arr, g_arr, stp),
+                      "lsr_forward_preprocess_views_tb_async")
+            else:
+                check(L.lsr_forward_preprocess_views_rows_fused_async(n, int(r0), int(r1), s_arr, fi, o_arr, g_arr, fz,
+                                                                      stp),
+                      "lsr_forward_preprocess_views_rows_fused_async")
         if k > 0:
             check(count_fn(k, s_arr, fi, g_arr, ctypes.c_void_p(counts.data_ptr()), stp), count_what)
     else:
-        check(L.lsr_forward_preprocess_views_split_async(n, k, s_arr, fi, o_arr, g_arr,
-                                                         ctypes.c_void_p(counts.data_ptr() if k else 0), stp),
-              "lsr_forward_preprocess_views_split_async")
+        check(L.lsr_forward_preprocess_views_split_fused_async(n, k, s_arr, fi, o_arr, g_arr,
+                                                               ctypes.c_void_p(counts.data_ptr() if k else 0), fz, stp),
+              "lsr_forward_preprocess_views_split_fused_async")
     ev = torch.cuda.Event()
     ev.record(stream)
     late = None
diff --git a/4dlangsplat_amd/diff_gaussian_rasterization/_lib.py b/4dlangsplat_amd/diff_gaussian_rasterization/_lib.py
--- a/4dlangsplat_amd/diff_gaussian_rasterization/_lib.py
+++ b/4dlangsplat_amd/diff_gaussian_rasterization/_lib.py
@@ -48,6 +48,12 @@
                 ("dL_dlanguage_feature", ctypes.c_void_p), ("dL_dopacity", ctypes.c_void_p),
                 ("dL_dcov3D", ctypes.c_void_p), ("dL_dsh", ctypes.c_void_p), ("dL_dscales", ctypes.c_void_p),
                 ("dL_drotations", ctypes.c_void_p)]
+
+
+class PreprocessFused(ctypes.Structure):
+    _fields_ = [("language_split_out", ctypes.c_void_p), ("zero_rows", ctypes.c_void_p),
+                ("zero_row_floats", ctypes.c_int32), ("radii_max_accumulate", ctypes.c_int32),
+                ("radii_max_out", ctypes.c_void_p)]
 
 
 class DeformNet(ctypes.Structure):
@@ -156,6 +162,18 @@
                                                                ctypes.POINTER(FwdIn),
                                                                ctypes.POINTER(ctypes.POINTER(FwdOut)),
                                                                ctypes.POINTER(ctypes.c_void_p), ctypes.c_void_p]),
+    "lsr_forward_preprocess_views_split_fused_async": (ctypes.c_int, [ctypes.c_int32, ctypes.c_int32,
+                                                                      ctypes.POINTER(ctypes.POINTER(Settings)),
+                                                                      ctypes.POINTER(FwdIn),
+                                                                      ctypes.POINTER(ctypes.POINTER(FwdOut)),
+                                                                      ctypes.POINTER(ctypes.c_void_p), ctypes.c_void_p,
+                                                                      ctypes.POINTER(PreprocessFused), ctypes.c_void_p]),
+    "lsr_forward_preprocess_views_rows_fused_async": (ctypes.c_int, [ctypes.c_int32, ctypes.c_int32, ctypes.c_int32,
+                                                                     ctypes.POINTER(ctypes.POINTER(Settings)),
+                                                                     ctypes.POINTER(FwdIn),
+                                                                     ctypes.POINTER(ctypes.POINTER(FwdOut)),
+                                                                     ctypes.POINTER(ctypes.c_void_p),
+                                                                     ctypes.POINTER(PreprocessFused), ctypes.c_void_p]),
     "lsr_forward_depth_order_views_async": (ctypes.c_int, [ctypes.c_int32, ctypes.POINTER(ctypes.POINTER(Settings)),
                                                            ctypes.POINTER(FwdIn), ctypes.POINTER(ctypes.c_void_p),
                                                            ctypes.c_void_p, ctypes.c_void_p]),
diff --git a/4dlangsplat_amd/view_parallel.py b/4dlangsplat_amd/view_parallel.py
--- a/4dlangsplat_amd/view_parallel.py
+++ b/4dlangsplat_amd/view_parallel.py
@@ -206,7 +206,8 @@
 def native_view_renderer(scene, settings, grad_fn: Callable, deterministic: bool = False, overlap: bool = True,
                          batch_backward: bool = True, early_views=3, composite_batch: bool = True,
                          side_priority: int = 0, side_from_preprocess: bool = True, split_behind_counts: bool = True,
-                         fill_on_side: bool = False, order_on_side: bool = False, tile_bucket: bool = False):
+                         fill_on_side: bool = False, order_on_side: bool = False, tile_bucket: bool = False,
+                         fused_preprocess: bool = False):
     import diff_gaussian_rasterization as dgr
 
     lookahead = overlap == "lookahead"
@@ -241,7 +242,7 @@
             fn()
         return None
 
-    def batch_preprocess(v, before_wait=None, radii_out=None):
+    def batch_preprocess(v, before_wait=None, radii_out=None, bucket=None):
         views = [w for w in step_views[0] if w >= v] if step_views[0] is not None else [v]
         views = [w for w in views if has_view(w)] or [v]
         sizes = tuple(early_views) if isinstance(early_views, (tuple, list)) else (early_views,)
@@ -252,13 +253,22 @@
         to_side = fill_on_side and split_side
         late_order = order_on_side and split_side and not to_side
         waits = take_row_waits(scene.means3D.is_cuda)
+        fuse = (fused_preprocess and bucket is not None and split_behind_counts and not fill_on_side and not tile_bucket
+                and scene.means3D.is_cuda and bucket.C == 32 and bucket.P > 0 and radii_out is not None
+                and radii_out is bucket.radii and getattr(before_wait, "__self__", None) is bucket
+                and getattr(before_wait, "__func__", None) is GradBucket.zero_accumulated_)
+        if fuse:
+            fused_args = dict(fuse_split=True, zero_rows=bucket.views["language_feature"], radii_max_out=bucket.radii)
+            before_wait = radii_out = None
+        else:
+            fused_args = {}
         pfs = dgr.preprocess_views_native([settings[w] for w in views], scene.means3D, scene.opacities,
                                           shs=scene.shs, language_feature=scene.lang, scales=scene.scales,
                                           rotations=scene.rotations, split_behind_counts=split_behind_counts,
                                           split_stream=bin_side[0] if to_side else None,
                                           order_first=e0 if late_order else None,
                                           order_stream=bin_side[0] if late_order else None,
-                                          row_chunks=waits, tile_bucket=tile_bucket)
+                                          row_chunks=waits, tile_bucket=tile_bucket, **fused_args)
         fill_ready[0] = None
         if to_side:
             bin_side[0].wait_stream(torch.cuda.current_stream(scene.means3D.device))
@@ -334,7 +344,7 @@
         reduce_radii = bucket.radii is not None and scene.means3D.is_cuda
         fresh = views[0] not in pending
         if fresh:
-            batch_preprocess(views[0], before_wait, radii_out=bucket.radii if reduce_radii else None)
+            batch_preprocess(views[0], before_wait, radii_out=bucket.radii if reduce_radii else None, bucket=bucket)
         elif before_wait is not None:
             before_wait()
         pfs = [pending.pop(v) for v in views]
diff --git a/include/lsr.h b/include/lsr.h
--- a/include/lsr.h
+++ b/include/lsr.h
@@ -99,6 +99,22 @@
 int lsr_forward_preprocess_views_rows_async(int32_t n_views, int32_t row0, int32_t row1, const lsr_settings *const *s,
                                             const lsr_fwd_in *in, lsr_fwd_out *const *out, void *const *geom,
                                             lsr_stream_t stream);
+
+typedef struct lsr_preprocess_fused {
+    uint16_t *language_split_out;
+    float *zero_rows;
+    int32_t zero_row_floats;
+    int32_t radii_max_accumulate;
+    int32_t *radii_max_out;
+} lsr_preprocess_fused;
+int lsr_forward_preprocess_views_split_fused_async(int32_t n_views, int32_t n_ordered, const lsr_settings *const *s,
+                                                   const lsr_fwd_in *in, lsr_fwd_out *const *out, void *const *geom,
+                                                   uint32_t *host_counts, const lsr_preprocess_fused *fused,
+                                                   lsr_stream_t stream);
+int lsr_forward_preprocess_views_rows_fused_async(int32_t n_views, int32_t row0, int32_t row1,
+                                                  const lsr_settings *const *s, const lsr_fwd_in *in,
+                                                  lsr_fwd_out *const *out, void *const *geom,
+                                                  const lsr_preprocess_fused *fused, lsr_stream_t stream);
 int lsr_forward_depth_order_views_async(int32_t n_views, const lsr_settings *const *s, const lsr_fwd_in *in,
                                         void *const *geom, uint32_t *host_counts, lsr_stream_t stream);
 
```

Result: slower. 947.9 frames/s (-2.8%).
